# heli-sudoo/HKD-MPC

Hardware: AMD Instinct MI355X
Metric: batched DDP iters/sec (fwd+bwd), 4-phase 200-knot HKD fp64, batch=4096 (higher is better)
Workload: dtype f64

## Files before the change

### hkd-mpc_amd/csrc/hkd_model.h

```cpp
#pragma once

#ifndef __HIPCC__
#ifndef __host__
#define __host__
#define __device__
#endif
#endif
#include <math.h>

#define HKD_FN __host__ __device__ inline

namespace hkd {

constexpr int NX = 24;
constexpr int NU = 24;
constexpr int SE_N = 15;
constexpr int SW_N = 51;
constexpr int BW_N = 36;

constexpr double kMass = 8.9120000000000008e+00;
constexpr double kGravity = -9.8100000000000005e+00;
constexpr double kI00 = 2.7460779999999994e-02, kI01 = 1.0842021724855044e-19, kI02 = -1.2037062152420224e-35;
constexpr double kI11 = 2.4251579680000002e-01, kI22 = 2.6519357680000000e-01;
constexpr double kJ00 = 3.6415571589736352e+01, kJ01 = -1.6280111378663628e-17, kJ02 = 1.6528925920107902e-33;
// ... 96 lines not shown
    contact_moment(x, u, c, w);
#pragma unroll
    for (int i = 0; i < 3; ++i) tau[i] = R.r[0][i] * w[0] + R.r[1][i] * w[1] + R.r[2][i] * w[2];
    inertia_apply(om, Iw);
    rhs[0] = tau[0] - (om[1] * Iw[2] - om[2] * Iw[1]);
    rhs[1] = tau[1] - (om[2] * Iw[0] - om[0] * Iw[2]);
    rhs[2] = tau[2] - (om[0] * Iw[1] - om[1] * Iw[0]);
    inertia_inv_apply(rhs, acc);
#pragma unroll
    for (int i = 0; i < 3; ++i) xn[6 + i] = om[i] + dt * acc[i];
#pragma unroll
    for (int i = 0; i < 3; ++i) {
        double f = c[0] * u[i] + c[1] * u[3 + i] + c[2] * u[6 + i] + c[3] * u[9 + i];
        xn[9 + i] = x[9 + i] + dt * (f / kMass + (i == 2 ? kGravity : 0.0));
    }
#pragma unroll
    for (int l = 0; l < 4; ++l)
#pragma unroll
        for (int j = 0; j < 3; ++j) xn[12 + 3 * l + j] = x[12 + 3 * l + j] + (1.0 - c[l]) * u[12 + 3 * l + j] * dt;
}

HKD_FN void hkd_partial_compact(const double *x, const double *u, const double *c, double dt, double *Se,
                                double *Sw, double *Bw)
{
    const double *om = x + 6;
    const EulTrig tr = eul_trig(x);
    const double cp = tr.cp, sp = tr.sp, cr = tr.cr, sr = tr.sr;
    double a = sr * om[1] + cr * om[2], b = cr * om[1] - sr * om[2];
    const double icp = 1.0 / cp, tp = sp * icp;
    Se[0] = dt * a * sp * (icp * icp); Se[1] = dt * b * icp; Se[2] = 0.0; Se[3] = dt * sr * icp; Se[4] = dt * cr * icp;
    Se[5] = 0.0;                     Se[6] = -dt * a;     Se[7] = 0.0;     Se[8] = dt * cr;      Se[9] = -dt * sr;
    Se[10] = dt * a * icp * icp;     Se[11] = dt * tp * b; Se[12] = dt;    Se[13] = dt * sr * tp; Se[14] = dt * cr * tp;
    Rot R, Dy, Dp, Dr;
    rot_zyx(tr, R);
    rot_zyx_grad(tr, Dy, Dp, Dr);
    double w[3];
    contact_moment(x, u, c, w);
    double M[3][17];
#pragma unroll
    for (int i = 0; i < 3; ++i) {
        M[i][0] = Dy.r[0][i] * w[0] + Dy.r[1][i] * w[1] + Dy.r[2][i] * w[2];
        M[i][1] = Dp.r[0][i] * w[0] + Dp.r[1][i] * w[1] + Dp.r[2][i] * w[2];
        M[i][2] = Dr.r[0][i] * w[0] + Dr.r[1][i] * w[1] + Dr.r[2][i] * w[2];
#pragma unroll
        for (int q = 3; q < 17; ++q) M[i][q] = 0.0;
    }
#pragma unroll
    for (int l = 0; l < 4; ++l) {
        const double *f = u + 3 * l;
        double Sf[3][3] = {{0.0, -f[2], f[1]}, {f[2], 0.0, -f[0]}, {-f[1], f[0], 0.0}};
#pragma unroll
        for (int i = 0; i < 3; ++i)
#pragma unroll
            for (int k = 0; k < 3; ++k) {
                double t = c[l] * (R.r[0][i] * Sf[0][k] + R.r[1][i] * Sf[1][k] + R.r[2][i] * Sf[2][k]);
                M[i][3 + k] += t;
                if (k < 2) M[i][9 + 2 * l + k] = -t;
            }
    }
    double Iw[3];
    inertia_apply(om, Iw);
    const double Ssk[3][3] = {{0.0, -Iw[2], Iw[1]}, {Iw[2], 0.0, -Iw[0]}, {-Iw[1], Iw[0], 0.0}};
    const double So[3][3] = {{0.0, -om[2], om[1]}, {om[2], 0.0, -om[0]}, {-om[1], om[0], 0.0}};
    const double In[3][3] = {{kI00, kI01, kI02}, {kI01, kI11, 0.0}, {kI02, 0.0, kI22}};
#pragma unroll
    for (int i = 0; i < 3; ++i)
#pragma unroll
        for (int k = 0; k < 3; ++k)
            M[i][6 + k] = Ssk[i][k] - (So[i][0] * In[0][k] + So[i][1] * In[1][k] + So[i][2] * In[2][k]);
#pragma unroll
    for (int q = 0; q < 17; ++q) {
        double v[3] = {M[0][q], M[1][q], M[2][q]}, o[3];
        inertia_inv_apply(v, o);
        Sw[q] = dt * o[0]; Sw[17 + q] = dt * o[1]; Sw[34 + q] = dt * o[2];
    }
#pragma unroll
    for (int l = 0; l < 4; ++l) {
        double r0 = x[12 + 3 * l] - x[3], r1 = x[13 + 3 * l] - x[4], r2 = -x[5];
        double Sr[3][3] = {{0.0, -r2, r1}, {r2, 0.0, -r0}, {-r1, r0, 0.0}};
#pragma unroll
        for (int k = 0; k < 3; ++k) {
            double v[3], o[3];
#pragma unroll
            for (int i = 0; i < 3; ++i) v[i] = c[l] * (R.r[0][i] * Sr[0][k] + R.r[1][i] * Sr[1][k] + R.r[2][i] * Sr[2][k]);
            inertia_inv_apply(v, o);
            Bw[3 * l + k] = dt * o[0]; Bw[12 + 3 * l + k] = dt * o[1]; Bw[24 + 3 * l + k] = dt * o[2];
        }
    }
}

template <typename Emit>
HKD_FN void hkd_partial_emit(const double *x, const double *u, const double *c, double dt, Emit emit)
{
    const double *om = x + 6;
    const EulTrig tr = eul_trig(x);
    const double cp = tr.cp, sp = tr.sp, cr = tr.cr, sr = tr.sr;
    double a = sr * om[1] + cr * om[2], b = cr * om[1] - sr * om[2];
    const double icp = 1.0 / cp, tp = sp * icp;
    emit(0, 0, dt * a * sp * (icp * icp)); emit(0, 1, dt * b * icp); emit(0, 2, 0.0); emit(0, 3, dt * sr * icp);
    emit(0, 4, dt * cr * icp); emit(0, 5, 0.0); emit(0, 6, -dt * a); emit(0, 7, 0.0); emit(0, 8, dt * cr);
    emit(0, 9, -dt * sr); emit(0, 10, dt * a * icp * icp); emit(0, 11, dt * tp * b); emit(0, 12, dt);
    emit(0, 13, dt * sr * tp); emit(0, 14, dt * cr * tp);
    Rot R, Dy, Dp, Dr;
    rot_zyx(tr, R);
    rot_zyx_grad(tr, Dy, Dp, Dr);
    auto col = [&](const double (&v)[3], int q) {
        double o[3];
        inertia_inv_apply(v, o);
        emit(1, q, dt * o[0]); emit(1, 17 + q, dt * o[1]); emit(1, 34 + q, dt * o[2]);
    };
    {
        double w[3];
        contact_moment(x, u, c, w);
        double v[3];
#pragma unroll
        for (int i = 0; i < 3; ++i) v[i] = Dy.r[0][i] * w[0] + Dy.r[1][i] * w[1] + Dy.r[2][i] * w[2];
        col(v, 0);
#pragma unroll
        for (int i = 0; i < 3; ++i) v[i] = Dp.r[0][i] * w[0] + Dp.r[1][i] * w[1] + Dp.r[2][i] * w[2];
        col(v, 1);
#pragma unroll
        for (int i = 0; i < 3; ++i) v[i] = Dr.r[0][i] * w[0] + Dr.r[1][i] * w[1] + Dr.r[2][i] * w[2];
        col(v, 2);
    }
    auto tl = [&](int l, int i, int k) {
        const double *f = u + 3 * l;
        const double Sf[3][3] = {{0.0, -f[2], f[1]}, {f[2], 0.0, -f[0]}, {-f[1], f[0], 0.0}};
        return c[l] * (R.r[0][i] * Sf[0][k] + R.r[1][i] * Sf[1][k] + R.r[2][i] * Sf[2][k]);
    };
#pragma unroll
    for (int k = 0; k < 3; ++k) {
        double v[3] = {0.0, 0.0, 0.0};
#pragma unroll
        for (int l = 0; l < 4; ++l)
#pragma unroll
            for (int i = 0; i < 3; ++i) v[i] += tl(l, i, k);
        col(v, 3 + k);
    }
    {
        double Iw[3];
        inertia_apply(om, Iw);
        const double Ssk[3][3] = {{0.0, -Iw[2], Iw[1]}, {Iw[2], 0.0, -Iw[0]}, {-Iw[1], Iw[0], 0.0}};
        const double So[3][3] = {{0.0, -om[2], om[1]}, {om[2], 0.0, -om[0]}, {-om[1], om[0], 0.0}};
        const double In[3][3] = {{kI00, kI01, kI02}, {kI01, kI11, 0.0}, {kI02, 0.0, kI22}};
#pragma unroll
        for (int k = 0; k < 3; ++k) {
            double v[3];
#pragma unroll
            for (int i = 0; i < 3; ++i) v[i] = Ssk[i][k] - (So[i][0] * In[0][k] + So[i][1] * In[1][k] + So[i][2] * In[2][k]);
            col(v, 6 + k);
        }
    }
#pragma unroll
    for (int l = 0; l < 4; ++l)
#pragma unroll
        for (int k = 0; k < 2; ++k) {
            double v[3];
#pragma unroll
            for (int i = 0; i < 3; ++i) v[i] = -tl(l, i, k);
            col(v, 9 + 2 * l + k);
        }
#pragma unroll
    for (int l = 0; l < 4; ++l) {
        double r0 = x[12 + 3 * l] - x[3], r1 = x[13 + 3 * l] - x[4], r2 = -x[5];
        double Sr[3][3] = {{0.0, -r2, r1}, {r2, 0.0, -r0}, {-r1, r0, 0.0}};
#pragma unroll
        for (int k = 0; k < 3; ++k) {
            double v[3], o[3];
#pragma unroll
            for (int i = 0; i < 3; ++i) v[i] = c[l] * (R.r[0][i] * Sr[0][k] + R.r[1][i] * Sr[1][k] + R.r[2][i] * Sr[2][k]);
            inertia_inv_apply(v, o);
            emit(2, 3 * l + k, dt * o[0]); emit(2, 12 + 3 * l + k, dt * o[1]); emit(2, 24 + 3 * l + k, dt * o[2]);
        }
    }
}

HKD_FN void hkd_expand_colmajor(const double *Se, const double *Sw, const double *Bw, const double *c, double dt,
                                double *A, double *B)
{
    for (int i = 0; i < NX * NX; ++i) { A[i] = 0.0; B[i] = 0.0; }
    for (int i = 0; i < NX; ++i) A[i + NX * i] = 1.0;
    for (int r = 0; r < 3; ++r)
        for (int q = 0; q < 5; ++q) A[r + NX * se_col(q)] += Se[5 * r + q];
    for (int i = 0; i < 3; ++i) A[(3 + i) + NX * (9 + i)] = dt;
    for (int r = 0; r < 3; ++r)
        for (int q = 0; q < 17; ++q) A[(6 + r) + NX * sw_col(q)] += Sw[17 * r + q];
    for (int r = 0; r < 3; ++r)
        for (int k = 0; k < 12; ++k) B[(6 + r) + NX * k] = Bw[12 * r + k];
    for (int l = 0; l < 4; ++l)
        for (int j = 0; j < 3; ++j) {
            B[(9 + j) + NX * (3 * l + j)] = dt * c[l] / kMass;
            B[(12 + 3 * l + j) + NX * (12 + 3 * l + j)] = dt * (1.0 - c[l]);
        }
}

HKD_FN void foot_body_trig(int l, const double *tr, double *pb, double (*dpb)[3])
{
    double s = leg_side(l), f = leg_front(l);
    const double s0 = tr[0], c0 = tr[1], s1 = tr[2], c1 = tr[3], s12 = tr[4], c12 = tr[5];
    pb[0] = kHipX * f - kLower * s12 - kUpper * s1;
    pb[1] = kSideY * s + kAbad * s * c0 - kLower * s0 * c12 - kUpper * s0 * c1;
    pb[2] = kLower * c0 * c12 + kUpper * c0 * c1 + kAbad * s * s0;
    if (dpb) {
        dpb[0][0] = 0.0; dpb[0][1] = -kLower * c12 - kUpper * c1; dpb[0][2] = -kLower * c12;
        dpb[1][0] = -kAbad * s * s0 - kLower * c0 * c12 - kUpper * c0 * c1;
        dpb[1][1] = kLower * s0 * s12 + kUpper * s0 * s1; dpb[1][2] = kLower * s0 * s12;
        dpb[2][0] = -kLower * s0 * c12 - kUpper * s0 * c1 + kAbad * s * c0;
        dpb[2][1] = -kLower * c0 * s12 - kUpper * c0 * s1; dpb[2][2] = -kLower * c0 * s12;
    }
}

HKD_FN void foot_body(int l, const double *q, double *pb, double (*dpb)[3])
{
    double tr[6];
    sincos(q[0], &tr[0], &tr[1]);
    sincos(q[1], &tr[2], &tr[3]);
    sincos(q[1] + q[2], &tr[4], &tr[5]);
    foot_body_trig(l, tr, pb, dpb);
}

HKD_FN void hkd_foot_position(int l, const double *pos, const double *eul, const double *q, double *p)
{
    Rot R;
    rot_zyx(eul, R);
    double pb[3];
    foot_body(l, q, pb, nullptr);
    for (int i = 0; i < 3; ++i) p[i] = pos[i] + R.r[i][0] * pb[0] + R.r[i][1] * pb[1] + R.r[i][2] * pb[2];
}

HKD_FN void hkd_foot_jacobian(int l, const double *eul, const double *q, double *J)
{
    Rot R, Dy, Dp, Dr;
    const EulTrig tr = eul_trig(eul);
    rot_zyx(tr, R);
    rot_zyx_grad(tr, Dy, Dp, Dr);
    double pb[3], dpb[3][3];
    foot_body(l, q, pb, dpb);
    for (int i = 0; i < 54; ++i) J[i] = 0.0;
    for (int i = 0; i < 3; ++i) {
        J[18 * i + i] = 1.0;
        J[18 * i + 3] = Dy.r[i][0] * pb[0] + Dy.r[i][1] * pb[1] + Dy.r[i][2] * pb[2];
        J[18 * i + 4] = Dp.r[i][0] * pb[0] + Dp.r[i][1] * pb[1] + Dp.r[i][2] * pb[2];
        J[18 * i + 5] = Dr.r[i][0] * pb[0] + Dr.r[i][1] * pb[1] + Dr.r[i][2] * pb[2];
        for (int k = 0; k < 3; ++k)
            J[18 * i + 6 + 3 * l + k] = R.r[i][0] * dpb[0][k] + R.r[i][1] * dpb[1][k] + R.r[i][2] * dpb[2][k];
    }
}

__host__ __device__ __forceinline__ double hkd_foot_height_grad(int l, const double *x, double *hx)
{
    Rot R, Dy, Dp, Dr;
    const EulTrig tr = eul_trig(x);
    rot_zyx(tr, R);
    rot_zyx_grad(tr, Dy, Dp, Dr);
    double pb[3], dpb[3][3];
    foot_body(l, x + 12 + 3 * l, pb, dpb);
    if (hx) {
        for (int j = 0; j < NX; ++j) hx[j] = 0.0;
        hx[0] = Dy.r[2][0] * pb[0] + Dy.r[2][1] * pb[1] + Dy.r[2][2] * pb[2];
        hx[1] = Dp.r[2][0] * pb[0] + Dp.r[2][1] * pb[1] + Dp.r[2][2] * pb[2];
        hx[2] = Dr.r[2][0] * pb[0] + Dr.r[2][1] * pb[1] + Dr.r[2][2] * pb[2];
        hx[5] = 1.0;
        for (int k = 0; k < 3; ++k)
            hx[12 + 3 * l + k] = R.r[2][0] * dpb[0][k] + R.r[2][1] * dpb[1][k] + R.r[2][2] * dpb[2][k];
    }
    return x[5] + R.r[2][0] * pb[0] + R.r[2][1] * pb[1] + R.r[2][2] * pb[2];
}

HKD_FN double hkd_foot_height_grad_sparse(int l, const double *x, double *ge, double *gq)
{
    Rot R, Dy, Dp, Dr;
    const EulTrig tr = eul_trig(x);
    rot_zyx(tr, R);
    rot_zyx_grad(tr, Dy, Dp, Dr);
    double pb[3], dpb[3][3];
    foot_body(l, x + 12 + 3 * l, pb, dpb);
    ge[0] = Dy.r[2][0] * pb[0] + Dy.r[2][1] * pb[1] + Dy.r[2][2] * pb[2];
    ge[1] = Dp.r[2][0] * pb[0] + Dp.r[2][1] * pb[1] + Dp.r[2][2] * pb[2];
    ge[2] = Dr.r[2][0] * pb[0] + Dr.r[2][1] * pb[1] + Dr.r[2][2] * pb[2];
    for (int k = 0; k < 3; ++k) gq[k] = R.r[2][0] * dpb[0][k] + R.r[2][1] * dpb[1][k] + R.r[2][2] * dpb[2][k];
    return x[5] + R.r[2][0] * pb[0] + R.r[2][1] * pb[1] + R.r[2][2] * pb[2];
}

HKD_FN void hkd_resetmap(const double *x, const int *c, const int *cn, double *xn)
{
    for (int j = 0; j < NX; ++j) xn[j] = x[j];
#pragma unroll
    for (int l = 0; l < 4; ++l) {
        if (c[l] && !cn[l]) { xn[12 + 3 * l] = 0.0; xn[13 + 3 * l] = -0.8; xn[14 + 3 * l] = 1.7; }
        if (!c[l] && cn[l]) {
            double p[3];
            hkd_foot_position(l, x + 3, x, x + 12 + 3 * l, p);
            xn[12 + 3 * l] = p[0]; xn[13 + 3 * l] = p[1]; xn[14 + 3 * l] = 0.0 * p[2];
        }
    }
}

HKD_FN void hkd_resetmap_partial_row(const double *x, const int *c, const int *cn, int r, double *row)
{
    for (int j = 0; j < NX; ++j) row[j] = (j == r) ? 1.0 : 0.0;
    if (r < 12) return;
    int l = (r - 12) / 3, k = (r - 12) % 3;
    if (c[l] && !cn[l]) { row[r] = 0.0; return; }
    if (!c[l] && cn[l]) {
        row[r] = 0.0;
        if (k == 2) return;
        double J[54];
        hkd_foot_jacobian(l, x, x + 12 + 3 * l, J);
        for (int j = 0; j < 3; ++j) { row[j] = J[18 * k + 3 + j]; row[3 + j] = J[18 * k + j]; }
        for (int j = 0; j < 12; ++j) row[12 + j] = J[18 * k + 6 + j];
    }
}

}
```

### hkd-mpc_amd/csrc/hsddp_api.cpp

```cpp
#include <algorithm>
#include <cmath>
#include <cstddef>
#include <cstdio>
#include <cstdlib>
#include <cstring>

#include "hsddp_handle.h"
#include "hsddp_measure.h"
#include "hsddp_simulate.h"

using namespace hsddp;

static thread_local std::string g_err;

int hsddp::fail(int code, const std::string &msg)
{
    g_err = msg;
    return code;
}

extern "C" int hsddp_ref_fail(int code, const char *msg) { return fail(code, msg); }

extern "C" const char *hsddp_last_error(void) { return g_err.c_str(); }
extern "C" const char *hsddp_version(void) { return "hsddp-mi355x 0.1 (gfx950, fp64)"; }

static void fill_params(hsddp_handle h)
{
    h->slots_fresh = false;
    Params &p = h->p;
    const hsddp_problem_desc &ds = h->desc;
    const hsddp_options &o = h->opt;
    p.dt = ds.dt;
    p.dt_m = ds.dt / hkd::kMass;
    {
        const char *tr = std::getenv("HSDDP_TRACE");
        p.trace = (tr && tr[0] == '1') ? 1 : 0;
    }
    p.mu = ds.cparams.mu_fric;
    p.grf_delta = ds.cparams.grf_delta; p.grf_delta_min = ds.cparams.grf_delta_min; p.grf_eps = ds.cparams.grf_eps;
    p.td_sigma = ds.cparams.td_sigma; p.td_sigma_max = ds.cparams.td_sigma_max; p.td_lambda = ds.cparams.td_lambda;
    p.ground = ds.cparams.ground_height;
    const hsddp_hkd_weights &w = ds.weights;
    for (int j = 0; j < 3; ++j) { p.qbase[j] = w.q_eul[j]; p.qbase[3 + j] = w.q_pos[j]; p.qbase[6 + j] = w.q_omega[j]; p.qbase[9 + j] = w.q_v[j]; }
    p.q_qJ = w.q_qJ;
    for (int j = 0; j < 24; ++j) p.qf_scale[j] = w.qf_scale[j];
    p.qf_gain = w.qf_gain; p.r_grf = w.r_grf; p.r_qJd = w.r_qJd;
    for (int j = 0; j < 3; ++j) p.foot_w[j] = w.foot_w[j];
    p.foot_gain = w.foot_gain; p.foot_term_cost = w.foot_term_cost; p.foot_term_grad = w.foot_term_grad;
    p.alpha = o.alpha; p.gamma = o.gamma; p.update_penalty = o.update_penalty; p.update_relax = o.update_relax;
    p.update_regularization = o.update_regularization; p.update_ReB = o.update_ReB;
    p.cost_thresh = o.cost_thresh; p.tconstr_thresh = o.tconstr_thresh; p.pconstr_thresh = o.pconstr_thresh;
    p.feas_thresh = o.dynamics_feas_thresh; p.merit_scale = o.merit_scale; p.merit_offset = o.merit_offset;
    p.AL_active = o.AL_active; p.ReB_active = o.ReB_active; p.no_early_exit = o.no_early_exit;
    p.ms0 = o.MS ? 0 : 1;
    p.reb_uniform = o.update_ReB == 1.0 && o.update_relax == 1.0 && p.grf_delta >= p.grf_delta_min && h->reb_at_init;
    p.grf_inv_delta = 1.0 / p.grf_delta;
    p.grf_log_delta = std::log(p.grf_delta);
    int M = 0;
    if (o.update_regularization > 1) {
        double mu = 0;
        for (;;) {
            mu = std::fmax(mu * o.update_regularization, 1e-03);
            if (mu > 1e2) break;
            if (++M > 64) { M = 0; break; }
        }
    }
    p.retry_m = M;
    p.retry_cap = (M > 0 && M <= h->retry_m_alloc && !p.store_value && p.B >= 4) ? h->retry_cap_alloc : 0;
}

static int ensure_history(hsddp_handle h)
{
    const long need = std::max(1 + (long)std::max(0, h->opt.max_AL_iter) * std::max(0, h->opt.max_DDP_iter),
                               h->budgets_on ? 1 + h->bud_hist : 0L);
    if (h->hist && need <= h->p.hcap) return HSDDP_OK;
    const int cap = (int)std::min<long>(std::max<long>(need, 16), 1 << 20);
    float *nh = nullptr;
    HIPCHK(hipMalloc(&nh, (size_t)h->p.B * cap * 4 * sizeof(float)));
    HIPCHK(hipMemset(nh, 0, (size_t)h->p.B * cap * 4 * sizeof(float)));
    HIPCHK(hipStreamSynchronize(nullptr));
    if (h->hist) {
        HIPCHK(hipStreamSynchronize(h->stream));
        hipFree(h->hist);
        h->bytes -= (size_t)h->p.B * h->p.hcap * 4 * sizeof(float);
    }
    h->hist = nh;
    h->d.hist = nh;
    h->p.hcap = cap;
    h->bytes += (size_t)h->p.B * cap * 4 * sizeof(float);
    return HSDDP_OK;
}

extern "C" int hsddp_create(const hsddp_problem_desc *desc, hsddp_handle *out)
{
    if (!desc || !out) return fail(HSDDP_ERR_ARG, "null argument");
    if (desc->batch < 1 || desc->n_phases < 1 || desc->n_phases > HSDDP_MAX_PHASES || !(desc->dt > 0))
        return fail(HSDDP_ERR_ARG, "invalid batch / n_phases / dt");
    Layout L0;
    std::string why;
    if (int rc = build_layout(desc->n_phases, desc->horizons, nullptr, L0, why)) return fail(rc, why);
    int ndev = 0;
    if (hipGetDeviceCount(&ndev) != hipSuccess || ndev < 1)
        return fail(HSDDP_ERR_DEVICE, "no HIP device available (the solver has no CPU fallback)");
    if (desc->device < 0 || desc->device >= ndev) return fail(HSDDP_ERR_DEVICE, "device ordinal out of range");
    HIPCHK(hipSetDevice(desc->device));
    hsddp_handle h = new hsddp_handle_t();
    h->desc = *desc;
    hsddp_default_options(&h->opt);
    Params &p = h->p;
    p.B = desc->batch;
    p.Kc = control_slots(L0);
    p.ref_per_element = desc->ref_per_element ? 1 : 0;
    p.fp32 = desc->riccati_fp32 ? 1 : 0;
    h->Bref = p.ref_per_element ? p.B : 1;
    adopt_shared_layout(h, L0, nullptr);
    fill_params(h);
    h->S_cap = (size_t)p.Kc + HSDDP_MAX_PHASES;
    const size_t B = p.B, S = h->S_cap, Kc = p.Kc, P = HSDDP_MAX_PHASES, Br = h->Bref;
    Bufs &d = h->d;
    int *contacts; double *x0, *rx, *ru, *rf;
    int rc = 0;
    if ((rc = dalloc(h, contacts, B * (P + 1) * 4)) || (rc = dalloc(h, x0, B * NX)) || (rc = dalloc(h, rx, Br * S * NX)) ||
        (rc = dalloc(h, ru, Br * S * NX)) || (rc = dalloc(h, rf, Br * S * 12)) || (rc = dalloc(h, d.ref_t, REF_COLS * Br * S)) ||
        (rc = dalloc(h, d.X3, 3 * B * S * NX)) ||
        (rc = dalloc(h, d.D3, 3 * B * S * NX)) || (rc = dalloc(h, d.U3, 3 * B * Kc * NX)) || (rc = dalloc(h, d.sel, B)) ||
        (rc = dalloc(h, d.cf_u, B * Kc * 12)) || (rc = dalloc(h, d.cf_flag, B * Kc)) ||
        (rc = dalloc(h, d.dX, B * S * NX)) ||
        (rc = dalloc(h, d.dU, B * Kc * NX)) ||
        (rc = dalloc(h, d.du, B * Kc * NX)) || (rc = dalloc(h, d.dbg, B * 16)) ||
        (p.fp32 ? ((rc = dalloc(h, d.K32, B * Kc * KCW)) || (rc = dalloc(h, d.lq32, B * Kc * LQW32)) ||
                   (rc = dalloc(h, d.def32, B * S * NX)))
                : ((rc = dalloc(h, d.K, B * Kc * KCW)) || (rc = dalloc(h, d.lq, B * Kc * LQW)))) ||
        (rc = dalloc(h, d.term, B * P * TW)) || (rc = dalloc(h, d.reb_delta, B * Kc * 20)) ||
        (rc = dalloc(h, d.reb_eps, B * Kc * 20)) || (rc = dalloc(h, d.al_sigma, B * P * MTD * 4)) ||
        (rc = dalloc(h, d.al_lambda, B * P * MTD * 4)) || (rc = dalloc(h, d.td_mask, B * P * MTD)) ||
        (rc = dalloc(h, d.term_h, B * P * 4)) ||
        (rc = dalloc(h, d.slot_cost, B * S)) || (rc = dalloc(h, d.slot_feas, B * S)) || (rc = dalloc(h, d.slot_viol, B * S)) ||
        (rc = dalloc(h, d.slot_div, B * S)) || (rc = dalloc(h, d.el, B)) || (rc = dalloc(h, d.counter, 8)) || (rc = dalloc(h, d.ls_live, LS_LIVE)) ||
        (rc = dalloc(h, (Layout *&)d.lay, B)) || (rc = dalloc(h, (int *&)d.pairs, 2 * B + 2))) {
        hsddp_destroy(h);
        return rc;
    }
    d.contacts = contacts; d.x0 = x0; d.ref_x = rx; d.ref_u = ru; d.ref_foot = rf;
    d.ref_tw = Br * S;
    d.xs3 = B * S * NX;
    d.us3 = B * Kc * NX;
    d.rows3 = (int)(B * S);
    d.urows3 = (int)(B * Kc);
    {
        const char *seq = std::getenv("HSDDP_SEQUENTIAL_RETRY");
        const char *capenv = std::getenv("HSDDP_RETRY_CAP");
        const size_t per_elem = (size_t)std::max(1, p.retry_m) * Kc * (KCW * (p.fp32 ? 4 : 8) + NX * 8 + 4);
        size_t cap = std::min<size_t>(std::min<size_t>(128, B), std::max<size_t>(2, ((size_t)256 << 20) / per_elem));
        if (capenv && std::atoi(capenv) > 0) cap = std::min<size_t>(cap, (size_t)std::atoi(capenv));
        const size_t M = (seq && seq[0] == '1') ? 0 : p.retry_m, n = cap * M;
        if (M > 0) {
            void *rk;
            if ((rc = dalloc(h, d.retry_list, cap)) || (rc = dalloc(h, d.retry_count, 1)) ||
                (rc = dalloc(h, d.retry_flag, n)) || (rc = dalloc(h, d.retry_dU, n * Kc * NX)) ||
                (rc = dalloc(h, d.retry_dv, n)) ||
                (rc = p.fp32 ? dalloc(h, (float *&)rk, n * Kc * KCW) : dalloc(h, (double *&)rk, n * Kc * KCW))) {
                hsddp_destroy(h);
                return rc;
            }
            d.retry_K = rk;
            h->retry_cap_alloc = (int)cap;
            h->retry_m_alloc = (int)M;
            fill_params(h);
        }
    }
    if (hipStreamCreateWithFlags(&h->stream, hipStreamNonBlocking) != hipSuccess ||
        hipHostMalloc((void **)&h->host_counter, 16 * sizeof(int), 0) != hipSuccess) {
        hsddp_destroy(h);
        return fail(HSDDP_ERR_DEVICE, "stream / pinned allocation failed");
    }
    if ((rc = ensure_history(h))) {
        hsddp_destroy(h);
        return rc;
    }
    launch_init_params(p, d, h->stream);
    launch_reset_elements(p, d, h->stream);
    if (hipStreamSynchronize(h->stream) != hipSuccess) {
        hsddp_destroy(h);
        return fail(HSDDP_ERR_DEVICE, "kernel launch failed at create (is the library built for this GPU?)");
    }
    *out = h;
    return HSDDP_OK;
}

// ... 848 lines not shown
}

extern "C" int hsddp_download_trajectory(hsddp_handle h, double *Xbar, double *Ubar, double *K)
{
    if (!h) return fail(HSDDP_ERR_ARG, "null handle");
    HIPCHK(hipSetDevice(h->desc.device));
    HIPCHK(hipStreamSynchronize(h->stream));
    const size_t B = h->p.B, S = h->p.S, Kc = h->p.Kc;
    int rc;
    launch_normalize(h->p, h->d, h->stream);
    HIPCHK(hipStreamSynchronize(h->stream));
    if ((rc = d2h(Xbar, h->d.X3, B * S * NX * 8)) || (rc = d2h(Ubar, h->d.U3, B * Kc * NX * 8)))
        return rc;
    if (K && h->need_inputs)
        return fail(HSDDP_ERR_ARG, "the layout changed (hsddp_shift): call hsddp_update_problem before downloading K");
    if (K) {
        std::vector<double> kc(B * Kc * KCW);
        if (h->p.fp32) {
            std::vector<float> k32(B * Kc * KCW);
            if ((rc = d2h(k32.data(), h->d.K32, B * Kc * KCW * 4))) return rc;
            std::copy(k32.begin(), k32.end(), kc.begin());
        } else if ((rc = d2h(kc.data(), h->d.K, B * Kc * KCW * 8))) {
            return rc;
        }
        std::memset(K, 0, B * Kc * NN * sizeof(double));
        for (size_t b = 0; b < B; ++b)
            for (size_t k = 0; k < Kc; ++k)
                for (int q = 0; q < 12; ++q) {
                    const int u = coupled_control(h, b, k, q);
                    std::memcpy(K + ((b * Kc + k) * NX + u) * NX, &kc[((b * Kc + k) * 12 + q) * NX], NX * sizeof(double));
                }
    }
    return HSDDP_OK;
}

extern "C" int hsddp_debug_stamps(hsddp_handle h, unsigned long long *out)
{
    if (!h || !out) return fail(HSDDP_ERR_ARG, "null argument");
    HIPCHK(hipSetDevice(h->desc.device));
    HIPCHK(hipStreamSynchronize(h->stream));
    HIPCHK(hipMemcpy(out, h->d.dbg, h->p.B * 16 * sizeof(unsigned long long), hipMemcpyDeviceToHost));
    return HSDDP_OK;
}

extern "C" int hsddp_download_working(hsddp_handle h, double *X, double *U, double *Defect, double *dX, double *dU)
{
    if (!h) return fail(HSDDP_ERR_ARG, "null handle");
    HIPCHK(hipSetDevice(h->desc.device));
    HIPCHK(hipStreamSynchronize(h->stream));
    const size_t B = h->p.B, S = h->p.S, Kc = h->p.Kc;
    int rc;
    if ((rc = d2h(dX, h->d.dX, B * S * NX * 8)) || (rc = d2h(dU, h->d.dU, B * Kc * NX * 8)))
        return rc;
    if (X || U || Defect) {
        std::vector<int> sel(B);
        HIPCHK(hipMemcpy(sel.data(), h->d.sel, B * sizeof(int), hipMemcpyDeviceToHost));
        for (int q = 0; q < 3; ++q) {
            std::vector<double> xb(X ? B * S * NX : 0), ub(U ? B * Kc * NX : 0), db(Defect ? B * S * NX : 0);
            if ((rc = d2h(X ? xb.data() : nullptr, h->d.X3 + q * h->d.xs3, B * S * NX * 8)) ||
                (rc = d2h(U ? ub.data() : nullptr, h->d.U3 + q * h->d.us3, B * Kc * NX * 8)) ||
                (rc = d2h(Defect ? db.data() : nullptr, h->d.D3 + q * h->d.xs3, B * S * NX * 8)))
                return rc;
            for (size_t b = 0; b < B; ++b) {
                if (((sel[b] >> 2) & 3) != q) continue;
                if (X) std::copy(xb.begin() + b * S * NX, xb.begin() + (b + 1) * S * NX, X + b * S * NX);
                if (U) std::copy(ub.begin() + b * Kc * NX, ub.begin() + (b + 1) * Kc * NX, U + b * Kc * NX);
                if (Defect) std::copy(db.begin() + b * S * NX, db.begin() + (b + 1) * S * NX, Defect + b * S * NX);
            }
        }
    }
    return HSDDP_OK;
}

extern "C" int hsddp_download_references(hsddp_handle h, double *ref_x, double *ref_u, double *ref_foot)
{
    if (!h || !ref_x || !ref_u || !ref_foot) return fail(HSDDP_ERR_ARG, "null argument");
    HIPCHK(hipSetDevice(h->desc.device));
    HIPCHK(hipStreamSynchronize(h->stream));
    const size_t Br = h->Bref, S = h->p.S;
    int rc;
    if ((rc = d2h(ref_x, h->d.ref_x, Br * S * NX * 8)) || (rc = d2h(ref_u, h->d.ref_u, Br * S * NX * 8)) ||
        (rc = d2h(ref_foot, h->d.ref_foot, Br * S * 12 * 8)))
        return rc;
    return HSDDP_OK;
}

extern "C" int hsddp_download_element_info(hsddp_handle h, hsddp_element_info *info)
{
    if (!h || !info) return fail(HSDDP_ERR_ARG, "null argument");
    HIPCHK(hipSetDevice(h->desc.device));
    HIPCHK(hipStreamSynchronize(h->stream));
    std::vector<ElemState> el(h->p.B);
    HIPCHK(hipMemcpy(el.data(), h->d.el, h->p.B * sizeof(ElemState), hipMemcpyDeviceToHost));
    for (int b = 0; b < h->p.B; ++b) {
        const ElemState &e = el[b];
        info[b].cost = e.cost; info[b].feas = e.feas; info[b].merit = e.merit;
        info[b].max_tconstr = e.max_t; info[b].max_pconstr = e.max_p;
        info[b].iters = e.iters; info[b].outer_iters = e.outer_iters; info[b].status = e.status;
        info[b].n_ls_trials = e.n_ls;
    }
    return HSDDP_OK;
}

extern "C" int hsddp_download_solver_info(hsddp_handle h, int capacity, float *cost, float *dyn_feas,
                                          float *eqn_feas, float *ineq_feas, int *count)
{
    if (!h || capacity < 0) return fail(HSDDP_ERR_ARG, "null handle or negative capacity");
    HIPCHK(hipSetDevice(h->desc.device));
    HIPCHK(hipStreamSynchronize(h->stream));
    const int B = h->p.B, hc = h->p.hcap;
    std::vector<ElemState> el(B);
    HIPCHK(hipMemcpy(el.data(), h->d.el, B * sizeof(ElemState), hipMemcpyDeviceToHost));
    std::vector<float> hv((size_t)B * hc * 4);
    HIPCHK(hipMemcpy(hv.data(), h->d.hist, hv.size() * sizeof(float), hipMemcpyDeviceToHost));
    float *outs[4] = {cost, dyn_feas, eqn_feas, ineq_feas};
    for (int b = 0; b < B; ++b) {
        const int n = std::min(el[b].hist_n, std::min(hc, capacity));
        if (count) count[b] = n;
        for (int f = 0; f < 4; ++f) {
            if (!outs[f]) continue;
            float *o = outs[f] + (size_t)b * capacity;
            for (int k = 0; k < capacity; ++k) o[k] = k < n ? hv[((size_t)b * hc + k) * 4 + f] : 0.0f;
        }
    }
    return HSDDP_OK;
}



extern "C" int hsddp_download_lq(hsddp_handle h, double *A, double *Bm, double *l, double *lx, double *lu,
                                 double *lxx, double *luu)
{
    if (!h) return fail(HSDDP_ERR_ARG, "null handle");
    HIPCHK(hipSetDevice(h->desc.device));
    HIPCHK(hipStreamSynchronize(h->stream));
    const Params &p = h->p;
    const size_t B = p.B, Kc = p.Kc, S = p.S, W = p.fp32 ? LQW32 : LQW;
    std::vector<double> rec(B * Kc * W), cost(B * S);
    if (p.fp32) {
        std::vector<float> r32(B * Kc * W);
        HIPCHK(hipMemcpy(r32.data(), h->d.lq32, r32.size() * sizeof(float), hipMemcpyDeviceToHost));
        for (size_t q = 0; q < rec.size(); ++q) rec[q] = r32[q];
    } else {
        HIPCHK(hipMemcpy(rec.data(), h->d.lq, rec.size() * sizeof(double), hipMemcpyDeviceToHost));
    }
    if (l) HIPCHK(hipMemcpy(cost.data(), h->d.slot_cost, cost.size() * sizeof(double), hipMemcpyDeviceToHost));
    const double dt = p.dt;
    for (size_t b = 0; b < B; ++b)
        for (size_t kc = 0; kc < Kc; ++kc) {
            const double *r = rec.data() + (b * Kc + kc) * W;
            const int i = phase_of_control(layout_of(h, b), (int)kc);
            const int *c = h->contacts.data() + (b * (p.P + 1) + i) * 4;
            const size_t o = (b * Kc + kc);
            if (A) {
                double *a = A + o * NN;
                std::fill(a, a + NN, 0.0);
                for (int j = 0; j < NX; ++j) a[j * NX + j] = 1.0;
                for (int rr = 0; rr < 3; ++rr)
                    for (int q = 0; q < 5; ++q) a[rr * NX + hkd::se_col(q)] += r[LQ_SE + 5 * rr + q];
                for (int q = 0; q < 3; ++q) a[(3 + q) * NX + 9 + q] += dt;
                for (int rr = 0; rr < 3; ++rr)
                    for (int q = 0; q < 17; ++q) a[(6 + rr) * NX + hkd::sw_col(q)] += r[sw_at(rr, q)];
            }
            if (Bm) {
                double *bb = Bm + o * NN;
                std::fill(bb, bb + NN, 0.0);
                for (int rr = 0; rr < 3; ++rr)
                    for (int q = 0; q < 12; ++q) bb[(6 + rr) * NX + q] = r[bw_at(rr, q)];
                for (int lg = 0; lg < 4; ++lg)
                    for (int a = 0; a < 3; ++a) {
                        bb[(9 + a) * NX + 3 * lg + a] = dt * c[lg] / hkd::kMass;
                        bb[(12 + 3 * lg + a) * NX + 12 + 3 * lg + a] = dt * (1.0 - c[lg]);
                    }
            }
            Wts wr;
            weights_row(weights_of(h, b), wr);
            if (l) l[o] = cost[b * S + kc + i];
            if (lx) for (int j = 0; j < NX; ++j) lx[o * NX + j] = r[LQ_LX + j];
            if (lu) for (int j = 0; j < NX; ++j) lu[o * NX + j] = r[LQ_LU + j];
            if (lxx) {
                double *m = lxx + o * NN;
                std::fill(m, m + NN, 0.0);
                for (int j = 0; j < NX; ++j)
                    m[j * NX + j] = dt * (j < 12 ? wr.qbase[j] : wr.q_qJ * (1 - c[(j - 12) / 3]));
                for (int lg = 0; lg < 4; ++lg)
                    for (int a = 0; a < 3; ++a) {
                        const double w = c[lg] ? dt * (wr.foot_gain * wr.foot_w[a]) : 0.0;
                        const int pa = 3 + a, qa = 12 + 3 * lg + a;
                        m[pa * NX + pa] += w; m[qa * NX + qa] += w;
                        m[pa * NX + qa] -= w; m[qa * NX + pa] -= w;
                    }
            }
            if (luu) {
                double *m = luu + o * NN;
                std::fill(m, m + NN, 0.0);
                for (int j = 0; j < NX; ++j) m[j * NX + j] = dt * (j < 12 ? wr.r_grf : wr.r_qJd);
                static const int ix[3][3] = {{0, 1, 2}, {1, 3, 4}, {2, 4, 5}};
                for (int lg = 0; lg < 4; ++lg)
                    for (int a = 0; a < 3; ++a)
                        for (int e = 0; e < 3; ++e) m[(3 * lg + a) * NX + 3 * lg + e] += r[LQ_RB + 6 * lg + ix[a][e]];
            }
        }
    return HSDDP_OK;
}

extern "C" int hsddp_download_terminal(hsddp_handle h, double *Phi, double *Phix, double *Phixx, double *Px)
{
    if (!h) return fail(HSDDP_ERR_ARG, "null handle");
    HIPCHK(hipSetDevice(h->desc.device));
    HIPCHK(hipStreamSynchronize(h->stream));
    const Params &p = h->p;
    const size_t B = p.B, P = p.P;
    std::vector<double> term(B * P * TW), cost(B * p.S);
    HIPCHK(hipMemcpy(term.data(), h->d.term, term.size() * sizeof(double), hipMemcpyDeviceToHost));
    HIPCHK(hipMemcpy(cost.data(), h->d.slot_cost, cost.size() * sizeof(double), hipMemcpyDeviceToHost));
    for (size_t b = 0; b < B; ++b) {
        const Layout L = layout_of(h, b);
        for (size_t i = 0; i < P; ++i) {
            const double *t = term.data() + (b * P + i) * TW;
            const size_t o = b * P + i;
            if ((int)i >= L.P) {
                if (Phi) Phi[o] = 0;
                if (Phix) std::fill(Phix + o * NX, Phix + (o + 1) * NX, 0.0);
                if (Phixx) std::fill(Phixx + o * NN, Phixx + (o + 1) * NN, 0.0);
                if (Px) std::fill(Px + o * NN, Px + (o + 1) * NN, 0.0);
                continue;
            }
            if (Phi) Phi[o] = cost[b * p.S + L.s0[i] + L.N[i]];
            if (Phix) std::copy(t + TM_PHIX, t + TM_PHIX + NX, Phix + o * NX);
            if (Phixx) std::copy(t + TM_PHIXX, t + TM_PHIXX + NN, Phixx + o * NN);
            if (Px) {
                if ((int)i + 1 < L.P) std::copy(t + TM_PX, t + TM_PX + NN, Px + o * NN);
                else std::fill(Px + o * NN, Px + (o + 1) * NN, 0.0);
            }
        }
    }
    return HSDDP_OK;
}

extern "C" int hsddp_set_value_export(hsddp_handle h, int on)
{
    if (!h) return fail(HSDDP_ERR_ARG, "null handle");
    HIPCHK(hipSetDevice(h->desc.device));
    if (on && !h->value0) {
        const size_t n = (size_t)h->p.B * HSDDP_MAX_PHASES * (NX + NN);
        HIPCHK(hipMalloc(&h->value0, n * sizeof(double)));
        HIPCHK(hipMemset(h->value0, 0, n * sizeof(double)));
        HIPCHK(hipStreamSynchronize(nullptr));
        h->bytes += n * sizeof(double);
        h->d.value0 = h->value0;
    }
    h->p.store_value = on ? 1 : 0;
    fill_params(h);
    return HSDDP_OK;
}

extern "C" int hsddp_download_value(hsddp_handle h, double *G, double *H)
{
    if (!h) return fail(HSDDP_ERR_ARG, "null handle");
    if (!h->value0 || !h->p.store_value) return fail(HSDDP_ERR_ARG, "value export is off (hsddp_set_value_export)");
    HIPCHK(hipSetDevice(h->desc.device));
    HIPCHK(hipStreamSynchronize(h->stream));
    const size_t B = h->p.B, P = h->p.P;
    std::vector<double> v(B * P * (NX + NN));
    HIPCHK(hipMemcpy(v.data(), h->value0, v.size() * sizeof(double), hipMemcpyDeviceToHost));
    for (size_t o = 0; o < B * P; ++o) {
        const bool live = (int)(o % P) < layout_of(h, o / P).P;
        const double *s = v.data() + o * (NX + NN);
        if (G) { if (live) std::copy(s, s + NX, G + o * NX); else std::fill(G + o * NX, G + (o + 1) * NX, 0.0); }
        if (H) { if (live) std::copy(s + NX, s + NX + NN, H + o * NN); else std::fill(H + o * NN, H + (o + 1) * NN, 0.0); }
    }
    return HSDDP_OK;
}

extern "C" int hsddp_synchronize(hsddp_handle h)
{
    if (!h) return fail(HSDDP_ERR_ARG, "null handle");
    HIPCHK(hipStreamSynchronize(h->stream));
    return HSDDP_OK;
}

extern "C" size_t hsddp_device_bytes(hsddp_handle h) { return h ? h->bytes : 0; }

static int check_launch()
{
    HIPCHK(hipGetLastError());
    return HSDDP_OK;
}

extern "C" int hsddp_hkd_dynamics(const double *x, const double *u, const double *c, double dt, double *xn, int n,
                                  void *stream)
{
    if (!x || !u || !c || !xn || n < 0) return fail(HSDDP_ERR_ARG, "bad argument");
    if (n) launch_model_dynamics(x, u, c, dt, xn, n, (hipStream_t)stream);
    return check_launch();
}
extern "C" int hsddp_hkd_dynamics_partial(const double *x, const double *u, const double *c, double dt, double *A,
                                          double *B, int n, void *stream)
{
    if (!x || !u || !c || !A || !B || n < 0) return fail(HSDDP_ERR_ARG, "bad argument");
    if (n) launch_model_partial(x, u, c, dt, A, B, n, (hipStream_t)stream);
    return check_launch();
}
extern "C" int hsddp_hkd_foot_position(const double *x, const int *leg, double *p, int n, void *stream)
{
    if (!x || !leg || !p || n < 0) return fail(HSDDP_ERR_ARG, "bad argument");
    if (n) launch_model_foot(x, leg, p, nullptr, n, (hipStream_t)stream);
    return check_launch();
}
extern "C" int hsddp_hkd_state(const hsddp_robot_state *states, const int *contact, double *x, int n, void *stream)
{
    if (!states || !contact || !x || n < 0) return fail(HSDDP_ERR_ARG, "bad argument");
    if (n) launch_hkd_state(states, contact, 4, x, n, (hipStream_t)stream);
    return check_launch();
}
extern "C" int hsddp_hkd_foot_jacobian(const double *x, const int *leg, double *J, int n, void *stream)
{
    if (!x || !leg || !J || n < 0) return fail(HSDDP_ERR_ARG, "bad argument");
    if (n) launch_model_foot(x, leg, nullptr, J, n, (hipStream_t)stream);
    return check_launch();
}
extern "C" int hsddp_hkd_resetmap(const double *x, const int *c, const int *cn, double *xn, int n, void *stream)
{
    if (!x || !c || !cn || !xn || n < 0) return fail(HSDDP_ERR_ARG, "bad argument");
    if (n) launch_model_reset(x, c, cn, xn, nullptr, n, (hipStream_t)stream);
    return check_launch();
}
extern "C" int hsddp_hkd_resetmap_partial(const double *x, const int *c, const int *cn, double *Px, int n,
                                          void *stream)
{
    if (!x || !c || !cn || !Px || n < 0) return fail(HSDDP_ERR_ARG, "bad argument");
    if (n) launch_model_reset(x, c, cn, nullptr, Px, n, (hipStream_t)stream);
    return check_launch();
}

static Params plugin_params(const hsddp_hkd_weights &w, double dt)
{
    Params p{};
    p.dt = dt;
    for (int j = 0; j < 3; ++j) { p.qbase[j] = w.q_eul[j]; p.qbase[3 + j] = w.q_pos[j]; p.qbase[6 + j] = w.q_omega[j]; p.qbase[9 + j] = w.q_v[j]; }
    p.q_qJ = w.q_qJ;
    for (int j = 0; j < 24; ++j) p.qf_scale[j] = w.qf_scale[j];
    p.qf_gain = w.qf_gain; p.r_grf = w.r_grf; p.r_qJd = w.r_qJd;
    for (int j = 0; j < 3; ++j) p.foot_w[j] = w.foot_w[j];
    p.foot_gain = w.foot_gain; p.foot_term_cost = w.foot_term_cost; p.foot_term_grad = w.foot_term_grad;
    return p;
}
extern "C" int hsddp_hkd_running_cost(const double *x, const double *u, const int *c, const double *xr, const double *ur,
                                      const double *pf, const hsddp_hkd_weights *w, double dt, int terms, double *l,
                                      double *lx, double *lu, double *lxx, double *luu, int n, void *stream)
{
    if (!x || !u || !c || !xr || !ur || !pf || !w || n < 0 || (terms & ~3)) return fail(HSDDP_ERR_ARG, "bad argument");
    if (n) launch_model_running_cost(plugin_params(*w, dt), x, u, c, xr, ur, pf, terms, l, lx, lu, lxx, luu, n,
// ... 56 lines not shown
```

### hkd-mpc_amd/csrc/hsddp_internal.h

```cpp
#pragma once

#include <hip/hip_runtime.h>
#include <cstddef>
#include "hkd_model.h"
#include "hsddp_phases.h"

namespace hsddp {

constexpr int NX = 24;
constexpr int NN = 576;
constexpr int LS_LIVE = 128;
constexpr int MTD = 4;
constexpr int TD_PENDING = 0x10;
constexpr int KCW = 12 * 24;

constexpr int LQ_SE = 0;
constexpr int LQ_SW = 16;
constexpr int LQ_BW = 68;
constexpr int LQ_LX = 104;
constexpr int LQ_LU = 128;
constexpr int LQ_RB = 152;
constexpr int LQW = 176;
constexpr int LQW32 = 192;
constexpr int sw_at(int r, int q) { return LQ_SW + 3 * q + r; }
constexpr int bw_at(int r, int k) { return LQ_BW + 3 * k + r; }
static_assert(LQ_SE + 15 < LQ_SW && LQ_SW + 51 < LQ_BW && LQ_BW + 36 == LQ_LX && LQ_LX + 24 == LQ_LU &&
              LQ_LU + 24 == LQ_RB && LQ_RB + 24 == LQW, "record layout");

constexpr int MAX_REG_ATTEMPTS = 64;

constexpr int TM_PHIX = 0;
constexpr int TM_PHIXX = 32;
constexpr int TM_PX = TM_PHIXX + NN;
constexpr int TW = TM_PX + NN;
static_assert(TM_PHIXX % 16 == 0 && TM_PX % 16 == 0 && TW % 16 == 0, "terminal record lines");


struct Params {
    int B, P, S, Kc;
    int N[MAXP], s0[MAXP], k0[MAXP];
    int ref_per_element;
    double dt, dt_m , mu, grf_delta, grf_delta_min, grf_eps, td_sigma, td_sigma_max, td_lambda, ground;
    double qbase[12], q_qJ, qf_scale[24], qf_gain, r_grf, r_qJd, foot_w[3], foot_gain, foot_term_cost, foot_term_grad;
    double alpha, gamma, update_penalty, update_relax, update_regularization, update_ReB;
    double cost_thresh, tconstr_thresh, pconstr_thresh, feas_thresh, merit_scale, merit_offset;
    int AL_active, ReB_active, no_early_exit;
    int reb_uniform;
    double grf_inv_delta, grf_log_delta;
    int lq_slots;
    int fp32;
    int ss[MAXP];
    int has_tail;
    int retry_cap, retry_m;
    int hcap;
    int elem_layout;
    int n_pairs;
    int store_value;
    int ms0;
    int trace;
};

struct Wts {
    double qbase[12], q_qJ, qf_scale[24], qf_gain, r_grf, r_qJd, foot_w[3], foot_gain, foot_term_cost, foot_term_grad;
    double pad[2];
};
static_assert(sizeof(Wts) == 48 * sizeof(double), "Wts: three 128-byte lines");
static_assert(offsetof(Params, foot_term_grad) - offsetof(Params, qbase) == offsetof(Wts, foot_term_grad),
              "Wts: Params' weight fields in Params' order");

struct RetryEntry {
    int b, pad;
    double reg;
};

constexpr int TD_STALE = 0x20;

struct ElemState {
    double cost, feas, merit, merit_rho, dV1, dV2, reg;
    double max_t, max_p, max_t_prev, max_p_prev, cost_prev, merit_prev, feas_prev;
    int done, inner_done, ls_active, accepted, status, iters, outer_iters, n_ls;
    int hist_n;
    int ovr, td_stale;
    int inner_n;
};
static_assert(sizeof(ElemState) == 160, "ElemState: 14 doubles and 12 ints, no padding left");


struct Bufs {
    const int *contacts;
    const double *x0;
    const double *ref_x, *ref_u, *ref_foot;
    double *ref_t;
    size_t ref_tw;
    double *X3, *D3, *dX;
    double *U3, *dU, *du;
    size_t xs3, us3;
    int rows3, urows3;
    int *sel;
    double *cf_u;
    int *cf_flag;
    double *K, *lq, *term;
    double *reb_delta, *reb_eps, *al_sigma, *al_lambda, *term_h;
    int *td_mask;
    double *slot_cost, *slot_feas, *slot_viol;
    int *slot_div;
    float *lq32, *K32, *def32;
    ElemState *el;
    int *counter;
    int *ls_live;
    RetryEntry *retry_list;
    int *retry_count, *retry_flag;
    void *retry_K;
    double *retry_dU;
    double *retry_dv;
    unsigned long long *dbg;
    float *hist;
    const Layout *lay;
    const int *pairs;
    double *value0;
};


void launch_lq(const Params &p, const Bufs &d, const double *terrain, const Wts *weights, hipStream_t st);

void launch_riccati(const Params &p, const Bufs &d, const Wts *weights, hipStream_t st);
void launch_lin_rollout(const Params &p, const Bufs &d, const Wts *weights, hipStream_t st);

void launch_rollout(const Params &p, const Bufs &d, double eps, int last, int init, int tix, const int *budget,
                    const double *terrain, const Wts *weights, hipStream_t st);
void launch_decide(const Params &p, const Bufs &d, double eps, int last, int init, int tix, const int *budget,
                   const double *terrain, const Wts *weights, hipStream_t st);

void launch_normalize(const Params &p, const Bufs &d, hipStream_t st);
void launch_reset_working(const Params &p, const Bufs &d, hipStream_t st);
void launch_outer_begin(const Params &p, const Bufs &d, const int *budget, hipStream_t st);
void launch_reb_update(const Params &p, const Bufs &d, const double *terrain, hipStream_t st);
void launch_outer_end(const Params &p, const Bufs &d, const int *budget, hipStream_t st);
void launch_reset_elements(const Params &p, const Bufs &d, hipStream_t st);
void launch_init_params(const Params &p, const Bufs &d, hipStream_t st);
void launch_resolve_td(const Params &p, const Bufs &d, hipStream_t st);
void launch_upload_td(const Params &p, const Bufs &d, const int *legs, hipStream_t st);
constexpr int REF_COLS = 24 + 24 + 12;
void launch_ref_columns(const Params &p, const Bufs &d, int Bref, hipStream_t st);
void launch_count(const Params &p, const Bufs &d, int which, hipStream_t st);
void launch_stat_sums(const Params &p, const Bufs &d, hipStream_t st);
void launch_broadcast(double *dst, const double *src, size_t n, size_t copies, hipStream_t st);

void launch_model_dynamics(const double *x, const double *u, const double *c, double dt, double *xn, int n,
                           hipStream_t st);
void launch_model_partial(const double *x, const double *u, const double *c, double dt, double *A, double *B,
                          int n, hipStream_t st);
void launch_model_foot(const double *x, const int *leg, double *p, double *J, int n, hipStream_t st);
void launch_model_reset(const double *x, const int *c, const int *cn, double *xn, double *Px, int n,
                        hipStream_t st);
void launch_model_running_cost(const Params &p, const double *x, const double *u, const int *c, const double *xr,
                               const double *ur, const double *pf, int terms, double *l, double *lx, double *lu,
                               double *lxx, double *luu, int n, hipStream_t st);
void launch_model_terminal_cost(const Params &p, const double *x, const int *c, const double *xr, const double *pf,
                                int terms, double *Phi, double *Phix, double *Phixx, int n, hipStream_t st);
void launch_model_grf(const double *u, const int *c, double mu, double *g, double *gu, int n, hipStream_t st);
void launch_model_touchdown(const double *x, const int *c, const int *cn, double ground, double *h, double *hx, int n,
                            hipStream_t st);

}
```

### hkd-mpc_amd/csrc/hsddp_linear.hip

```cpp
#include "hsddp_wave.h"
#include "hsddp_dispatch.h"

namespace hsddp {

using namespace hkd;

constexpr int HC = 12;

#ifndef HSDDP_STAMPS
#define HSDDP_STAMPS 0
#endif
#if HSDDP_STAMPS
struct LinStamps {
    unsigned long long st[8], tprev;
};
DEV LinStamps &lin_stamps()
{
    __shared__ LinStamps s;
    return s;
}
#define LSTAMP(n)                                                                             \
    do {                                                                                      \
        __builtin_amdgcn_sched_barrier(0);                                                    \
        unsigned long long t_;                                                                \
        asm volatile("s_waitcnt lgkmcnt(0)\n\ts_memtime %0\n\ts_waitcnt lgkmcnt(0)" : "=s"(t_)::"memory"); \
        __builtin_amdgcn_sched_barrier(0);                                                    \
        if (threadIdx.x == 0) {                                                               \
            if ((n) > 0) lin_stamps().st[n] += t_ - lin_stamps().tprev;                       \
            lin_stamps().tprev = t_;                                                          \
        }                                                                                     \
    } while (0)
#else
#define LSTAMP(n) \
    do {          \
    } while (0)
#endif

template <typename real> struct Prec;
template <> struct Prec<double> {
    static constexpr int LQS = LQW;
    static DEV const double *lq(const Bufs &d) { return d.lq; }
    static DEV double *K(const Bufs &d) { return d.K; }
    static DEV const double *def(const Bufs &d, int b) { return kdbuf(work_buf(d, b)); }
};
template <> struct Prec<float> {
    static constexpr int LQS = LQW32;
    static DEV const float *lq(const Bufs &d) { return d.lq32; }
    static DEV float *K(const Bufs &d) { return d.K32; }
    static DEV const float *def(const Bufs &d, int) { return d.def32; }
};

template <typename real>
struct PhaseConst {
    int c[4];
    int cmask;
    real bv[4];
    real bq[4];
};

template <typename real>
DEV void load_phase(const Params &p, const Bufs &d, const size_t (&b)[2], int hf, int i, PhaseConst<real> &pc)
{
    typedef const __attribute__((address_space(4))) int cint;
    cint *c0 = (cint *)(d.contacts + (b[0] * (p.P + 1) + i) * 4), *c1 = (cint *)(d.contacts + (b[1] * (p.P + 1) + i) * 4);
    pc.cmask = 0;
#pragma unroll
    for (int l = 0; l < 4; ++l) {
        const int a0 = c0[l], a1 = c1[l];
        pc.c[l] = hf ? a1 : a0;
        pc.cmask |= (pc.c[l] != 0) << l;
        pc.bv[l] = pc.c[l] ? (real)p.dt_m : (real)0;
        pc.bq[l] = pc.c[l] ? (real)0 : (real)p.dt;
    }
}

template <typename real>
struct LxxRow {
    real diag, xq[4], xp;
};

template <typename real>
DEV int contact(const PhaseConst<real> &pc, int l) { return (pc.cmask >> l) & 1; }

template <typename T>
DEV T pick4(const T (&a)[4], int i)
{
    return i == 0 ? a[0] : i == 1 ? a[1] : i == 2 ? a[2] : a[3];
}

template <int N>
DEV double pick(const double (&a)[N], int i)
{
    double e[N];
#pragma unroll
    for (int k = 0; k < N; ++k) {
        e[k] = a[k];
        asm volatile("" : "+s"(e[k]));
    }
    double v = e[0];
#pragma unroll
    for (int k = 1; k < N; ++k) v = i == k ? e[k] : v;
    return v;
}

template <typename real, typename WT>
DEV void lxx_row(const Params &p, const WT &ww, const PhaseConst<real> &pc, int r, LxxRow<real> &L)
{
    auto at = [&](const auto &a, int i) {
        if constexpr (std::is_same_v<WT, Params>) return pick(a, i);
        else return a[i];
    };
    L.diag = 0.0; L.xp = 0.0;
#pragma unroll
    for (int l = 0; l < 4; ++l) L.xq[l] = 0.0;
    if (r >= NX) return;
    double dg = p.dt * (r < 12 ? at(ww.qbase, r) : ww.q_qJ * (1 - contact(pc, (r - 12) / 3)));
    if (r >= 3 && r < 6) {
        const double fw = p.dt * (ww.foot_gain * at(ww.foot_w, r - 3));
#pragma unroll
        for (int l = 0; l < 4; ++l) {
            const double w = pc.c[l] ? fw : 0.0;
            dg += w;
            L.xq[l] = -w;
        }
    } else if (r >= 12) {
        const int m = r - 12;
        const double w = contact(pc, m / 3) ? p.dt * (ww.foot_gain * at(ww.foot_w, m % 3)) : 0.0;
        dg += w;
        L.xp = -w;
    }
    L.diag = dg;
}

template <typename real>
struct LinImg {
    static constexpr int K = 0;
    static constexpr int LQ = K + KCW * (int)sizeof(real);
    static constexpr int D = LQ + Prec<real>::LQS * (int)sizeof(real);
    static constexpr int DU = D + NX * (int)sizeof(real);
    static constexpr int END = DU + NX * 8;
    static constexpr int NI = (END / 16 + 63) / 64;
    static_assert(LQ % 16 == 0 && D % 16 == 0 && DU % 16 == 0 && END % 16 == 0 && (NI == 4 || NI == 3), "16-byte pieces");
};
template <typename real>
struct LinBuf {
    alignas(16) char v[2][LinImg<real>::NI * 1024];
};
constexpr int LZ = 31;
template <typename real>
struct LinVec {
    real dx[2][32], du[2][32];
    real zero[64];
};

template <typename real>
struct LinSrc {
    using I = LinImg<real>;
    const char *p[2][I::NI];
    unsigned step[I::NI];

    static DEV int piece(int j, int lane)
    {
        const int o = 16 * (64 * j + lane);
        return o < I::END ? o : I::END - 16;
    }
    DEV void init(const Params &pr, const Bufs &d, const size_t (&b)[2], int s, int kc, int lane)
    {
#pragma unroll
        for (int j = 0; j < I::NI; ++j) {
            const int o = piece(j, lane);
            step[j] = o < I::LQ ? KCW * sizeof(real) : o < I::D ? Prec<real>::LQS * sizeof(real) : o < I::DU ? NX * sizeof(real) : NX * 8;
#pragma unroll
            for (int h = 0; h < 2; ++h) {
                const size_t kq = b[h] * pr.Kc + kc;
                const char *base = o < I::LQ ? (const char *)(Prec<real>::K(d) + kq * KCW) - I::K
                                 : o < I::D  ? (const char *)(Prec<real>::lq(d) + kq * Prec<real>::LQS) - I::LQ
                                 : o < I::DU ? (const char *)(Prec<real>::def(d, (int)b[h]) + (b[h] * pr.S + s + 1) * NX) - I::D
                                             : (const char *)(d.dU + kq * NX) - I::DU;
                p[h][j] = base + o;
            }
        }
    }
    DEV void advance()
    {
#pragma unroll
        for (int j = 0; j < I::NI; ++j) {
            p[0][j] += step[j];
            p[1][j] += step[j];
        }
    }
};

template <typename real>
DEV void lin_fetch(LinBuf<real> &buf, const LinSrc<real> &src)
{
#pragma unroll
    for (int h = 0; h < 2; ++h)
#pragma unroll
        for (int j = 0; j < LinImg<real>::NI; ++j)
            lds_dma16_nt(src.p[h][j], (unsigned)(size_t)(buf.v[h] + 1024 * j));
}

template <int W>
DEV void vm_wait()
{
    if constexpr (W == 0) asm volatile("s_waitcnt vmcnt(0)" ::: "memory");
    else if constexpr (W == 2) asm volatile("s_waitcnt vmcnt(2)" ::: "memory");
    else if constexpr (W == 6) asm volatile("s_waitcnt vmcnt(6)" ::: "memory");
    else if constexpr (W == 8) asm volatile("s_waitcnt vmcnt(8)" ::: "memory");
    else if constexpr (W == 10) asm volatile("s_waitcnt vmcnt(10)" ::: "memory");
    else if constexpr (W == 4) asm volatile("s_waitcnt vmcnt(4)" ::: "memory");
    else if constexpr (W == 12) asm volatile("s_waitcnt vmcnt(12)" ::: "memory");
    else static_assert(W < 0, "wait count");
}

template <int NI2>
DEV void vm_wait_n(int n)
{
    if (n == NI2 + 4) vm_wait<NI2 + 4>();
    else if (n == NI2 + 2) vm_wait<NI2 + 2>();
    else if (n == NI2) vm_wait<NI2>();
    else if (n == 4) vm_wait<4>();
    else if (n == 2) vm_wait<2>();
    else vm_wait<0>();
}

template <typename real>
struct LinRow {
    PhaseConst<real> pc;
    LxxRow<real> lx;
    real ru;
    bool cpl;
    int krow0;
    bool use_se, use_sw, use_rb;
    int se0, sw0, rb0, rbi[3];
    real c3;
    int i3;
    real cx[4];
    int ix[4];
    real cu[4];
    int iu[4];
    real cq;
    int iru;
};

template <typename real>
DEV void lin_row(const Params &p, LinRow<real> &R, int r)
{
    const int rr = r < NX ? r : 0;
    R.use_se = r < 3;
    R.use_sw = r >= 6 && r < 9;
    R.use_rb = r < 12;
    R.se0 = LQ_SE + 5 * (r < 3 ? r : 0);
    R.sw0 = r >= 6 && r < 9 ? r - 6 : 0;
    R.rb0 = LQ_RB + 6 * ((r < 12 ? r : 0) / 3);
    const int a = (r < 12 ? r : 0) % 3;
#pragma unroll
    for (int b = 0; b < 3; ++b) R.rbi[b] = a == 0 ? b : a == 1 ? (b == 0 ? 1 : b == 1 ? 3 : 4) : (b == 0 ? 2 : b == 1 ? 4 : 5);
    R.iru = r < 12 ? 3 * (r / 3) : LZ;
    R.c3 = (r >= 3 && r < 6) ? (real)p.dt : (real)0;
    R.i3 = (r >= 3 && r < 6) ? r + 6 : LZ;
#pragma unroll
    for (int l = 0; l < 4; ++l) {
        const bool pos = r >= 3 && r < 6, q = r >= 12 && r < NX;
        R.cx[l] = pos ? R.lx.xq[l] : (q && l == 0) ? R.lx.xp : (real)0;
        R.ix[l] = pos ? 12 + 3 * l + r - 3 : (q && l == 0) ? 3 + (r - 12) % 3 : LZ;
        const bool v = r >= 9 && r < 12;
        R.cu[l] = v ? R.pc.bv[l] : (real)0;
        R.iu[l] = v ? 3 * l + r - 9 : LZ;
    }
    R.cq = (r >= 12 && r < NX) ? pick4(R.pc.bq, (rr - 12) / 3) : (real)0;
}

template <typename real>
struct LinOut {
    double *du, *dx;
    real vu, vx;
    int n;
    int nprev;
    bool ust;
};

template <typename real>
DEV void lin_push(LinOut<real> &out, real du, real nx)
{
    out.vu = du;
    out.vx = nx;
    out.n = 1;
}

template <typename real>
DEV int lin_store_pending(bool go, bool st, LinOut<real> &out)
{
    if (!go || out.n == 0) return 0;
    out.n = 0;
    if (st) {
        if (out.ust) *out.du = (double)out.vu;
        *out.dx = (double)out.vx;
    }
    out.du += NX;
    out.dx += NX;
    return 2;
}

template <typename real>
DEV void lin_knot(const Params &p, LinVec<real> &S, LinBuf<real> &cur, LinBuf<real> &nxt, bool more, bool pend,
                  LinSrc<real> &src, const LinRow<real> &R, bool st, LinOut<real> &out, real &dx, real &q1s, real &q2s)
{
    using I = LinImg<real>;
    constexpr int NI2 = 2 * I::NI;
    const int lane = threadIdx.x, r = lane & 31, hf = lane >> 5;
    const bool rowl = r < NX;
    const int rr = rowl ? r : 0;
    LSTAMP(0);
    if (more) {
        src.advance();
        lin_fetch(nxt, src);
    }
    const int ns = lin_store_pending(pend, st, out);
    vm_wait_n<NI2>(out.nprev + (more ? NI2 : 0) + ns);
    out.nprev = ns;
    LSYNC();
    LSTAMP(1);
    const char *img = cur.v[hf];
    const real *kimg = (const real *)(img + I::K), *lq = (const real *)(img + I::LQ), *dd = (const real *)(img + I::D);
    const double *dUi = (const double *)(img + I::DU);
    real *sdxv = S.dx[hf], *sduv = S.du[hf];
    const real *kp = R.cpl ? kimg + R.krow0 : S.zero;
    const real *sep = R.use_se ? lq + R.se0 : S.zero, *swp = R.use_sw ? lq + LQ_SW + R.sw0 : S.zero;
    const real *bwp = R.use_sw ? lq + LQ_BW + R.sw0 : S.zero, *rbp = R.use_rb ? lq + R.rb0 : S.zero;
    const real *lxp = rowl ? lq + LQ_LX : S.zero, *lup = rowl ? lq + LQ_LU : S.zero;
    real krow[NX], cse[5], csw[17], cbw[12], crb[3];
#pragma unroll
    for (int c = 0; c < NX; ++c) krow[c] = kp[c];
    const real dUr = (real)dUi[rr];
#pragma unroll
    for (int q = 0; q < 5; ++q) cse[q] = sep[5 * 0 + q];
#pragma unroll
    for (int q = 0; q < 17; ++q) csw[q] = swp[3 * q];
    const real ddr = (rowl ? dd : S.zero)[rr], lxr = lxp[rr], lur = lup[rr];
    if (rowl) sdxv[r] = dx;
    real dxa, dxb;
    row_pair(dx, dxa, dxb);
    asm volatile("" : "+v"(dxa), "+v"(dxb));
    asm volatile("s_nop 1");
    pin(krow);
    real k0 = 0, k1 = 0;
    static_for<HC>([&](auto C) {
        constexpr int c = C, c1 = HC + C;
        bfma<c>(k0, dxa, krow[c]);
        if constexpr (c1 < 16) bfma<c1>(k1, dxa, krow[c1]);
        else bfma<c1 - 16>(k1, dxb, krow[c1]);
    });
    const real du = dUr + (k0 + k1);
    LSTAMP(2);
    SFENCE();
#pragma unroll
    for (int q = 0; q < 12; ++q) cbw[q] = bwp[3 * q];
#pragma unroll
    for (int b = 0; b < 3; ++b) crb[b] = rbp[R.rbi[b]];
    if (rowl) sduv[r] = du;
    const real x3 = sdxv[R.i3];
    real xc[4];
#pragma unroll
    for (int l = 0; l < 4; ++l) xc[l] = sdxv[R.ix[l]];
    pin(cse);
    pin(csw);
    real se = 0, sw = 0;
    static_for<5>([&](auto Q) { bfma<se_col(Q)>(se, dxa, cse[Q]); });
    static_for<17>([&](auto Q) {
        constexpr int col = sw_col(Q);
        if constexpr (col < 16) bfma<col>(sw, dxa, csw[Q]);
        else bfma<col - 16>(sw, dxb, csw[Q]);
    });
    real dua, dub;
    row_pair(du, dua, dub);
    asm volatile("" : "+v"(dua), "+v"(dub));
    asm volatile("s_nop 1");
    pin(cbw);
    real bw = 0;
    static_for<12>([&](auto C) { bfma<C>(bw, dua, cbw[C]); });
    (void)dub;
    LSYNC();
    LSTAMP(3);
    real uc[4], ur[3];
#pragma unroll
    for (int l = 0; l < 4; ++l) uc[l] = sduv[R.iu[l]];
#pragma unroll
    for (int b = 0; b < 3; ++b) ur[b] = sduv[R.iru < LZ ? R.iru + b : LZ];
    const real sdx = (se + sw) + R.c3 * x3;
    real lxd = R.lx.diag * dx;
#pragma unroll
    for (int l = 0; l < 4; ++l) lxd += R.cx[l] * xc[l];
    real bdu = bw;
#pragma unroll
    for (int l = 0; l < 4; ++l) bdu += R.cu[l] * uc[l];
    bdu += R.cq * du;
    const real lud = R.ru * du + (crb[0] * ur[0] + crb[1] * ur[1] + crb[2] * ur[2]);
    const real nx = rowl ? ((dx + sdx) + bdu) + ddr : (real)0;
    q1s += lxr * dx + lur * du;
    q2s += dx * lxd + du * lud;
    lin_push(out, du, nx);
    dx = nx;
    LSYNC();
    LSTAMP(4);
}

template <typename real, bool EL, typename... WP>
__global__ __launch_bounds__(64, 2) void k_lin_rollout(Params p, Bufs d, WP... wp)
{
    const auto wt = terrain_of(wp...);
    __shared__ LinVec<real> S;
    __shared__ LinBuf<real> B0;
    __shared__ LinBuf<real> B1;
    const int lane = threadIdx.x, r = lane & 31, hf = lane >> 5;
    size_t eb[2];
    bool valid;
    if constexpr (EL) {
        const int e0 = d.pairs[2 * blockIdx.x], e1 = d.pairs[2 * blockIdx.x + 1];
        eb[0] = e0;
        eb[1] = e1 >= 0 ? e1 : e0;
        valid = hf == 0 || e1 >= 0;
    } else {
        const int e0 = 2 * blockIdx.x, e1 = e0 + 1;
        eb[0] = e0;
        eb[1] = e1 < p.B ? e1 : e0;
        valid = hf == 0 || e1 < p.B;
    }
    const size_t b = hf ? eb[1] : eb[0];
    ElemState &E = d.el[b];
    const bool act = valid && !E.done && !E.inner_done;
    if (!__builtin_amdgcn_ballot_w64(act)) return;
    const bool rowl = r < NX, st = rowl && act;
    const int rr = rowl ? r : 0;
    const real *defg = Prec<real>::def(d, (int)b);
    S.zero[lane] = 0;
    S.dx[hf][r] = 0;
    S.du[hf][r] = 0;
#if HSDDP_STAMPS
    if (lane < 8) lin_stamps().st[lane] = 0;
#endif
    __syncthreads();
    real v1 = 0, v2 = 0, dx = 0;
    const auto LY = layout_of<EL>(d, (int)eb[0]);
    const int P = LY.P();
    LinOut<real> out{};
    for (int i = 0; i < P; ++i) {
        const int N = LY.N(i), s0 = LY.s0(i), k0 = LY.k0(i);
        LinSrc<real> src;
        src.init(p, d, eb, s0, k0, lane);
        lin_fetch(B0, src);
        out.nprev = 0;
        LinRow<real> R;
        load_phase(p, d, eb, hf, i, R.pc);
        if (i > 0) {
            const double *Px = d.term + (b * p.P + (i - 1)) * TW + TM_PX;
            if (rowl) S.dx[hf][r] = dx;
            LSYNC();
            real a = 0;
            if (rowl)
                for (int j = 0; j < NX; ++j) a += (real)Px[r * NX + j] * S.dx[hf][j];
            dx = a;
            LSYNC();
        } else {
            dx = 0;
        }
        if (rowl) dx = dx + defg[(b * p.S + s0) * NX + r];
        if (st) d.dX[(b * p.S + s0) * NX + r] = dx;
        lxx_row(p, wt.w(p, b), R.pc, r, R.lx);
        R.ru = rowl ? (real)(p.dt * r_diag(wt.w(p, b), r)) : (real)0;
        const bool stl = contact(R.pc, (rr % HC) / 3) != 0;
        R.cpl = rowl && (rr < HC ? stl : !stl);
        R.krow0 = (rr % HC) * NX;
        lin_row(p, R, r);
        out.ust = true;
        out.du = d.du + (b * p.Kc + k0) * NX + rr;
        out.dx = d.dX + (b * p.S + s0 + 1) * NX + rr;
        real q1s = 0, q2s = 0;
        for (int k = 0; k < N; k += 2) {
            lin_knot(p, S, B0, B1, k + 1 < N, k > 0, src, R, st, out, dx, q1s, q2s);
            if (k + 1 < N) lin_knot(p, S, B1, B0, k + 2 < N, true, src, R, st, out, dx, q1s, q2s);
        }
        lin_store_pending(true, st, out);
        const double *rec = d.term + (b * p.P + i) * TW;
        if (rowl) S.dx[hf][r] = dx;
        LSYNC();
        if (rowl) {
            q1s += (real)rec[TM_PHIX + r] * dx;
            real a = 0;
            for (int c = 0; c < NX; ++c) a += (real)rec[TM_PHIXX + r * NX + c] * S.dx[hf][c];
            q2s += dx * a;
        }
        v1 += half_sum(q1s);
        v2 += half_sum(q2s);
        LSYNC();
    }
#if HSDDP_STAMPS
    __syncthreads();
    if (lane < 8) d.dbg[(size_t)__builtin_amdgcn_readfirstlane((int)eb[1]) * 16 + 8 + lane] += lin_stamps().st[lane];
#endif
    if (r == 0 && act) merit_step(p, E, v1, v2);
}
void launch_lin_rollout(const Params &p, const Bufs &d, const Wts *weights, hipStream_t st)
{
    const dim3 g((unsigned)(p.elem_layout ? p.n_pairs : (p.B + 1) / 2));
    with_flags_table([&](auto f32, auto el, auto... wp) {
        using real = std::conditional_t<decltype(f32)::value, float, double>;
        hipLaunchKernelGGL((k_lin_rollout<real, decltype(el)::value>), g, dim3(64), 0, st, p, d, wp...);
    }, weights, p.fp32, p.elem_layout);
}

}
```

### hkd-mpc_amd/csrc/hsddp_lq.hip

```cpp
#include "hsddp_device.h"
#include "hsddp_dispatch.h"

namespace hsddp {

using namespace hkd;

#ifndef FWD_MINB
#define FWD_MINB 2
#endif

template <typename T> constexpr int LQ_STG = 128 / (int)sizeof(T) + 1;

template <typename T>
DEV void lq_flush(T *wl, const long *ridx, T *lq, int ldw, int lane, int OFF, int N)
{
    wave_sync();
    using T2 = std::conditional_t<std::is_same_v<T, float>, float2, double2>;
    const unsigned long long m = __ballot(1);
    const int na = __popcll(m), rank = __popcll(m & ((1ull << lane) - 1));
    for (int q = rank; q < 64 * (N / 2); q += na) {
        const int r = q / (N / 2), jp = q % (N / 2);
        const long rr = ridx[r];
        if (rr >= 0) {
            T2 w;
            w.x = wl[r * LQ_STG<T> + 2 * jp];
            w.y = wl[r * LQ_STG<T> + 2 * jp + 1];
            *reinterpret_cast<T2 *>(lq + rr * ldw + OFF + 2 * jp) = w;
        }
    }
    wave_sync();
}

#ifndef HSDDP_TERM_TPW
#define HSDDP_TERM_TPW 2
#endif
constexpr int TERM_TPW = HSDDP_TERM_TPW, TERM_TL = 64 / TERM_TPW;
struct TermLds {
    double sx[NX], shx[4][NX], scoef[4][2], sh[4], sxr[NX], spf[12], ssl[2 * MTD * 4];
    double sdw[NX + 12];
    double spx[12 * (NX + 1)];
    int sc[4], scn[4], smask[MTD];
};
static_assert(TERM_TL >= NX && TERM_TL >= 2 * MTD * 4 && TERM_TL >= 16, "terminal lane roles");

template <bool EL, typename TR>
DEV void terminal_task(const Params &p, const Bufs &d, const TR &terr, TermLds &S, int task, int t)
{
    const int b = task / p.P, i = task % p.P;
    const ElemState &E = d.el[b];
    if (E.done || E.inner_done) return;
    const auto L = layout_of<EL>(d, b);
    const int P = L.P();
    if (i >= P) return;
    double *sx = S.sx, (*shx)[NX] = S.shx, (*scoef)[2] = S.scoef, *sh = S.sh, *sxr = S.sxr, *spf = S.spf, *ssl = S.ssl;
    int *sc = S.sc, *scn = S.scn, *smask = S.smask;
    const int s = L.s0(i) + L.N(i);
    const double *xr = ref_ptr(p, d.ref_x, b, s, NX), *pf = ref_ptr(p, d.ref_foot, b, s, 12);
    if (t < NX) {
        sx[t] = xbuf(d, work_buf(d, b))[((size_t)b * p.S + s) * NX + t];
        sxr[t] = xr[t];
    }
    if (t < 2 * MTD * 4) ssl[t] = (t < MTD * 4 ? d.al_sigma : d.al_lambda)[((size_t)b * p.P + i) * MTD * 4 + (t & (MTD * 4 - 1))];
    constexpr int MK = TERM_TL - MTD;
    if (t >= MK) smask[t - MK] = d.td_mask[((size_t)b * p.P + i) * MTD + t - MK];
    if (t >= 4 && t < 16) spf[t - 4] = pf[t - 4];
    if (t < 4) {
        const int *cc = d.contacts + ((size_t)b * (p.P + 1) + i) * 4;
        sc[t] = cc[t]; scn[t] = cc[4 + t];
    }
    wave_sync();
    double *spx = S.spx;
    const bool bnd = i < P - 1;
    for (int e = t; e < 4 * NX; e += TERM_TL) (&shx[0][0])[e] = 0.0;
    if (bnd)
        for (int e = t; e < 12 * (NX + 1); e += TERM_TL) spx[e] = (e / (NX + 1) + 12 == e % (NX + 1)) ? 1.0 : 0.0;
    double *strig = S.sdw;
    unsigned need = td_union(smask);
#pragma unroll
    for (int l = 0; l < 4; ++l) need |= (bnd && touchdown(sc, scn, l)) ? 1u << l : 0u;
    if (need && t < 15) {
        const int m = t - 3;
        const double a = t < 3 ? sx[t] : m % 3 == 2 ? sx[11 + m] + sx[12 + m] : sx[12 + m];
        sincos(a, &strig[2 * t], &strig[2 * t + 1]);
    }
    wave_sync();
    if (t < 4) {
        const int l = t;
        const bool tdc = (td_union(smask) >> l) & 1, tdr = touchdown(sc, scn, l);
        double h = 0.0;
        if (tdc || (bnd && tdr)) {
            Rot R, Dy, Dp, Dr;
            const EulTrig tr{strig[1], strig[0], strig[3], strig[2], strig[5], strig[4]};
            rot_zyx(tr, R);
            rot_zyx_grad(tr, Dy, Dp, Dr);
            double pb[3], dpb[3][3];
            foot_body_trig(l, strig + 6 + 6 * l, pb, dpb);
            shx[l][0] = Dy.r[2][0] * pb[0] + Dy.r[2][1] * pb[1] + Dy.r[2][2] * pb[2];
            shx[l][1] = Dp.r[2][0] * pb[0] + Dp.r[2][1] * pb[1] + Dp.r[2][2] * pb[2];
            shx[l][2] = Dr.r[2][0] * pb[0] + Dr.r[2][1] * pb[1] + Dr.r[2][2] * pb[2];
#pragma unroll
            for (int k = 0; k < 3; ++k) shx[l][12 + 3 * l + k] = R.r[2][0] * dpb[0][k] + R.r[2][1] * dpb[1][k] + R.r[2][2] * dpb[2][k];
            shx[l][5] = 1.0;
            h = (sx[5] + R.r[2][0] * pb[0] + R.r[2][1] * pb[1] + R.r[2][2] * pb[2]) - terr.ground(p, b, i);
            if (!tdc) {
                h = 0.0;
#pragma unroll
                for (int j = 0; j < NX; ++j) shx[l][j] = 0.0;
            }
            if (bnd && tdr) {
#pragma unroll
                for (int k = 0; k < 3; ++k) {
                    double *row = spx + (3 * l + k) * (NX + 1);
                    row[12 + 3 * l + k] = 0.0;
                    if (k == 2) continue;
                    row[0] = Dy.r[k][0] * pb[0] + Dy.r[k][1] * pb[1] + Dy.r[k][2] * pb[2];
                    row[1] = Dp.r[k][0] * pb[0] + Dp.r[k][1] * pb[1] + Dp.r[k][2] * pb[2];
                    row[2] = Dr.r[k][0] * pb[0] + Dr.r[k][1] * pb[1] + Dr.r[k][2] * pb[2];
                    row[3 + k] = 1.0;
#pragma unroll
                    for (int m = 0; m < 3; ++m)
                        row[12 + 3 * l + m] = R.r[k][0] * dpb[0][m] + R.r[k][1] * dpb[1][m] + R.r[k][2] * dpb[2][m];
                }
            }
        } else if (bnd && sc[l] && !scn[l]) {
#pragma unroll
            for (int k = 0; k < 3; ++k) spx[(3 * l + k) * (NX + 2) + 12] = 0.0;
        }
        double c0 = 0.0, c1 = 0.0;
        if (tdc && p.AL_active)
            for (int q = 0; q < MTD; ++q)
                if ((smask[q] >> l) & 1) {
                    const double sg = ssl[4 * q + l], lm = ssl[MTD * 4 + 4 * q + l];
                    const double hq = (smask[q] & TD_STALE) ? 0.0 : h;
                    c0 += sg * hq + lm;
                    c1 += sg * (1 + hq) + lm;
                }
        scoef[l][0] = c0;
        scoef[l][1] = c1;
        sh[l] = h;
    }
    wave_sync();
    const auto &w = terr.w(p, b);
    const auto &kp = terr.wk(b);
    double *rec = d.term + ((size_t)b * p.P + i) * TW;
    if (t == 0) {
        double tv;
        d.slot_cost[(size_t)b * p.S + s] = terminal_cost_h(p, w, sc, sx, sxr, spf, smask, ssl, ssl + MTD * 4, sh, tv);
    }
    if (t < NX) {
        const int j = t;
        double v = kp.qf_gain * kp.qf_scale[j] * q_diag(kp, sc, j) * (sx[j] - sxr[j]);
        if (j >= 3 && j < 6) {
            for (int l = 0; l < 4; ++l) {
                int m = 3 * l + (j - 3);
                double e = (sx[12 + m] - sx[j]) - (spf[m] - sxr[j]);
                v += -(w.foot_term_grad * sc[l] * foot_weight(kp, sc, m) * e);
            }
        } else if (j >= 12) {
            int m = j - 12, l = m / 3;
            double e = (sx[j] - sx[3 + m % 3]) - (spf[m] - sxr[3 + m % 3]);
            v += w.foot_term_grad * sc[l] * foot_weight(kp, sc, m) * e;
        }
        for (int l = 0; l < 4; ++l) v += scoef[l][0] * shx[l][j];
        rec[TM_PHIX + j] = v;
    }
    auto fw = [&](int l, int j) { return w.foot_term_grad * sc[l] * sc[l] * foot_weight(kp, sc, 3 * l + j); };
    double *sdd = S.sdw, *scw = S.sdw + NX;
    if (t < NX) {
        const int r = t;
        double v = kp.qf_gain * kp.qf_scale[r] * q_diag(kp, sc, r);
        if (r >= 3 && r < 6) {
            for (int l = 0; l < 4; ++l) v += fw(l, r - 3);
        } else if (r >= 12) {
            v += fw((r - 12) / 3, (r - 12) % 3);
        }
        sdd[r] = v;
    }
    if (t < 12) scw[t] = fw(t / 3, t % 3);
    wave_sync();
    bool use[4];
#pragma unroll
    for (int l = 0; l < 4; ++l) use[l] = scoef[l][1] != 0.0;
    int r = t / NX, cidx = t % NX;
    for (int e = t; e < NN; e += TERM_TL) {
        double v = 0.0;
        if (r == cidx)
            v = sdd[r];
        else if (r >= 3 && r < 6 && cidx >= 12 && (cidx - 12) % 3 == r - 3)
            v = -scw[cidx - 12];
        else if (cidx >= 3 && cidx < 6 && r >= 12 && (r - 12) % 3 == cidx - 3)
            v = -scw[r - 12];
#pragma unroll
        for (int l = 0; l < 4; ++l)
            if (use[l]) v += scoef[l][1] * (shx[l][r] * shx[l][cidx]);
        rec[TM_PHIXX + e] = v;
        if (bnd && r >= 12) rec[TM_PX + e] = spx[(r - 12) * (NX + 1) + cidx];
        r += TERM_TL / NX;
        cidx += TERM_TL % NX;
        if (cidx >= NX) {
            cidx -= NX;
            r += 1;
        }
    }
}

template <typename WT>
DEV void lq_lu_reb(const Params &p, const WT &w, double mu, const int *c, const double *u, const double *ovr, const double *ur, const double *dl,
                   const double *ep, double *lu, double *rb)
{
#pragma unroll
    for (int j = 0; j < NU; ++j) lu[j] = p.dt * r_diag(w, j) * (u[j] - ur[j]);
#pragma unroll
    for (int j = 0; j < 24; ++j) rb[j] = 0.0;
    auto reb = [&](auto uniform) {
        constexpr bool U = decltype(uniform)::value;
        const double inv_du = p.grf_inv_delta;
#pragma unroll
        for (int lg = 0; lg < 4; ++lg) {
            if (!c[lg]) continue;
            double gu[3] = {0, 0, 0}, hu[6] = {0, 0, 0, 0, 0, 0};
            const double f0 = grf_force(u, ovr, 3 * lg), f1 = grf_force(u, ovr, 3 * lg + 1), f2 = grf_force(u, ovr, 3 * lg + 2);
#pragma unroll
            for (int r = 0; r < 5; ++r) {
                double row[3], d1, d2;
                grf_row(mu, r, row);
                double g = row[0] * f0 + row[1] * f1 + row[2] * f2;
                const double dlr = U ? p.grf_delta : dl[5 * lg + r];
                reb_derivs(g, dlr, U ? inv_du : 1.0 / dlr, d1, d2);
                double e = U ? p.grf_eps : ep[5 * lg + r];
                for (int a = 0; a < 3; ++a) gu[a] += e * d1 * row[a];
                hu[0] += e * (d2 * row[0] * row[0]); hu[1] += e * (d2 * row[0] * row[1]);
                hu[2] += e * (d2 * row[0] * row[2]); hu[3] += e * (d2 * row[1] * row[1]);
                hu[4] += e * (d2 * row[1] * row[2]); hu[5] += e * (d2 * row[2] * row[2]);
            }
            for (int a = 0; a < 3; ++a) lu[3 * lg + a] += p.dt * gu[a];
            for (int a = 0; a < 6; ++a) rb[6 * lg + a] = p.dt * hu[a];
        }
    };
    if (p.ReB_active) {
        if (p.reb_uniform) reb(std::true_type{});
        else reb(std::false_type{});
    }
}

template <bool EL, typename TR>
DEV void terminal_wave(const Params &p, const Bufs &d, const TR &terr, TermLds *S, long wave, int lane)
{
    if (p.retry_cap > 0 && wave == 0 && lane == 0) *d.retry_count = 0;
    if (wave == 0)
        for (int t = lane; t < LS_LIVE; t += 64) d.ls_live[t] = 0;
    if (wave == 0 && lane < 4) d.counter[lane] = 0;
    const int h = lane / TERM_TL;
    const long task = wave * TERM_TPW + h;
    if (task < (long)p.B * p.P) terminal_task<EL>(p, d, terr, S[h], (int)task, lane % TERM_TL);
}

template <bool F32, bool EL, bool SLOTS, typename... TR>
__global__ __launch_bounds__(256, FWD_MINB) void k_lq(Params p, Bufs d, TR... tr)
{
    const auto terr = terrain_of(tr...);
    using T = std::conditional_t<F32, float, double>;
    constexpr size_t STG = sizeof(T) * 4 * 64 * LQ_STG<T>, TRM = 4 * TERM_TPW * sizeof(TermLds);
    __shared__ __attribute__((aligned(16))) char lds[STG > TRM ? STG : TRM];
    T (*stage)[64 * LQ_STG<T>] = reinterpret_cast<T (*)[64 * LQ_STG<T>]>(lds);
    __shared__ long sridx[4][64];
    const int lane = threadIdx.x & 63, w = threadIdx.x >> 6;
    constexpr bool BY_KNOT = !SLOTS && !F32;
    const long nunit = (long)p.B * (BY_KNOT ? p.Kc : p.S);
    const long nknot = (nunit + 255) / 256;
    if ((long)blockIdx.x >= nknot) {
        terminal_wave<EL>(p, d, terr, reinterpret_cast<TermLds *>(lds) + w * TERM_TPW, ((long)blockIdx.x - nknot) * 4 + w, lane);
        return;
    }
    sridx[w][lane] = -1;
    const long gid = (long)blockIdx.x * blockDim.x + threadIdx.x;
    if (gid >= nunit) return;
    const int b = (int)(gid / (BY_KNOT ? p.Kc : p.S));
    const ElemState &E = d.el[b];
    if (E.done || E.inner_done) return;
    const auto L = layout_of<EL>(d, b);
    int i, k, s;
    if constexpr (BY_KNOT) {
        const int kc0 = (int)(gid % p.Kc);
        knot_phase(L, kc0, i, k);
        if (k >= L.N(i)) return;
        s = L.s0(i) + k;
    } else {
        s = (int)(gid % p.S);
        if (s >= L.S()) return;
        slot_phase(L, s, i, k);
    }
    int c[4], cn[4];
    load_contacts(d, p, b, i, c, cn);
    double x[NX];
    const int wb = work_buf(d, b);
    const double *xg = xbuf(d, wb) + ((size_t)b * p.S + s) * NX;
#pragma unroll
    for (int j = 0; j < NX; ++j) x[j] = xg[j];
    const double *dg = dbuf(d, wb) + ((size_t)b * p.S + s) * NX;
    if (SLOTS) {
        double fs = 0.0;
#pragma unroll
        for (int j = 0; j < NX; ++j) fs += dg[j] * dg[j];
        d.slot_feas[(size_t)b * p.S + s] = fs;
    }
    if constexpr (F32) {
        float *d32 = d.def32 + ((size_t)b * p.S + s) * NX;
#pragma unroll
        for (int j = 0; j < NX; ++j) d32[j] = (float)dg[j];
    }
    const double *xr = ref_ptr(p, d.ref_x, b, s, NX), *pf = ref_ptr(p, d.ref_foot, b, s, 12);
    if (k == L.N(i)) return;
    const int kc = L.k0(i) + k;
    sridx[w][lane] = (long)b * p.Kc + kc;
    double u[NU];
    const double *ug = ubuf(d, wb) + ((size_t)b * p.Kc + kc) * NU;
#pragma unroll
    for (int j = 0; j < NU; ++j) u[j] = ug[j];
    const double *ovr = constraint_forces(d, E, b, kc);
    const double *ur = ref_ptr(p, d.ref_u, b, s, NU);
    const double *dl = d.reb_delta + ((size_t)b * p.Kc + kc) * 20, *ep = d.reb_eps + ((size_t)b * p.Kc + kc) * 20;
    const double mu = terr.mu(p, b, i);
    const auto &wr = terr.w(p, b);
    if (SLOTS) {
        double viol;
        d.slot_cost[(size_t)b * p.S + s] = running_cost(p, wr, mu, c, x, u, xr, ur, pf, dl, ep, viol, ovr);
    }

    T *lqT = F32 ? (T *)d.lq32 : (T *)d.lq;
    const int ldw = F32 ? LQW32 : LQW;
    double cd[4] = {(double)c[0], (double)c[1], (double)c[2], (double)c[3]};
    T *wl = stage[w];
    constexpr int W = 128 / (int)sizeof(T);
    auto col = [&](int pos) -> T & { return wl[lane * LQ_STG<T> + (pos & (W - 1))]; };
    auto put = [&](int pos, double v) {
        col(pos) = (T)v;
        if ((pos & (W - 1)) == W - 1) lq_flush(wl, sridx[w], lqT, ldw, lane, pos - (W - 1), W);
    };
    col(15) = 0;
    hkd_partial_emit(x, u, cd, p.dt, [&](int piece, int j, double v) {
        const int pos = piece == 0 ? LQ_SE + j : piece == 1 ? sw_at(j / 17, j % 17) : bw_at(j / 12, j % 12);
        col(pos) = (T)v;
        if (pos < 96 && ((pos & (W - 1)) == W - 1 || (W == 16 && pos == 14))) {
            lq_flush(wl, sridx[w], lqT, ldw, lane, pos & ~(W - 1), W);
            if (pos == 63) col(67) = 0;
        }
    });
    {
        double lx[NX];
#pragma unroll
        for (int j = 0; j < NX; ++j) lx[j] = p.dt * q_diag(wr, c, j) * (x[j] - xr[j]);
#pragma unroll
        for (int j = 0; j < 12; ++j) {
            double e = (x[12 + j] - x[3 + j % 3]) - (pf[j] - xr[3 + j % 3]);
            double v = p.dt * c[j / 3] * foot_weight(wr, c, j) * e;
            lx[3 + j % 3] += -v;
            lx[12 + j] += v;
        }
#pragma unroll
        for (int j = 0; j < NX; ++j) put(LQ_LX + j, lx[j]);
    }
    double lu[NU], rb[24];
    lq_lu_reb(p, wr, mu, c, u, ovr, ur, dl, ep, lu, rb);
#pragma unroll
    for (int j = 0; j < NU; ++j) put(LQ_LU + j, lu[j]);
#pragma unroll
    for (int j = 0; j < 24; ++j) put(LQ_RB + j, rb[j]);
    if constexpr (F32)
#pragma unroll
        for (int j = LQW; j < LQW32; ++j) put(j, 0.0);
}

template <bool EL, typename... TR>
__global__ __launch_bounds__(128, 4) void k_terminal(Params p, Bufs d, TR... tr)
{
    __shared__ TermLds S[2 * TERM_TPW];
    const int w = threadIdx.x >> 6;
    terminal_wave<EL>(p, d, terrain_of(tr...), S + w * TERM_TPW, (long)blockIdx.x * 2 + w, threadIdx.x & 63);
}

void launch_lq(const Params &p, const Bufs &d, const double *terrain, const Wts *weights, hipStream_t st)
{
    const unsigned nterm = blocks_for((long)p.B * p.P, 4 * TERM_TPW);
    const bool merged = nterm <= 256;
    const bool by_knot = !p.lq_slots && !p.fp32;
    if (!merged) {
        const unsigned nt2 = blocks_for((long)p.B * p.P, 2 * TERM_TPW);
        with_flags_tables([&](auto el, auto... tr) {
            hipLaunchKernelGGL(k_terminal<decltype(el)::value>, dim3(nt2), dim3(128), 0, st, p, d, tr...);
        }, terrain, weights, p.elem_layout);
    }
    const dim3 g(blocks_for((long)p.B * (by_knot ? p.Kc : p.S), 256) + (merged ? nterm : 0));
    with_flags_tables([&](auto f32, auto el, auto slots, auto... tr) {
        hipLaunchKernelGGL((k_lq<decltype(f32)::value, decltype(el)::value, decltype(slots)::value>), g, dim3(256), 0, st, p, d,
                           tr...);
    }, terrain, weights, p.fp32, p.elem_layout, p.lq_slots);
}

}
```

### hkd-mpc_amd/csrc/hsddp_solve.cpp

```cpp
#include <cstdlib>
#include <cstring>
#include <utility>

#include "hsddp_handle.h"

using namespace hsddp;

namespace {
struct Timer {
    hipStream_t st;
    bool on;
    std::vector<hipEvent_t> *pool;
    size_t used = 0;
    std::vector<std::pair<hipEvent_t, hipEvent_t>> ev[5];
    hipEvent_t pend = nullptr;
    hipEvent_t next()
    {
        if (used == pool->size()) {
            hipEvent_t e;
            hipEventCreate(&e);
            pool->push_back(e);
        }
        return (*pool)[used++];
    }
    void begin(int cat, hipEvent_t &e0)
    {
        if (!on) return;
        (void)cat;
        if (pend) {
            e0 = pend;
            pend = nullptr;
            return;
        }
        e0 = next();
        hipEventRecord(e0, st);
    }
    void cut() { pend = nullptr; }
    void end(int cat, hipEvent_t e0)
    {
        if (!on) return;
        hipEvent_t e1 = next();
        hipEventRecord(e1, st);
        ev[cat].push_back({e0, e1});
        pend = e1;
    }
    double total(int cat)
    {
        double t = 0;
        for (auto &pr : ev[cat]) {
            float ms = 0;
            hipEventElapsedTime(&ms, pr.first, pr.second);
            t += ms;
        }
        ev[cat].clear();
        return t;
    }
};
}

static int count_active(hsddp_handle h, int which, int &n)
{
    HIPCHK(hipMemsetAsync(h->d.counter, 0, 4 * sizeof(int), h->stream));
    launch_count(h->p, h->d, which, h->stream);
    HIPCHK(hipMemcpyAsync(h->host_counter, h->d.counter, 4 * sizeof(int), hipMemcpyDeviceToHost, h->stream));
    HIPCHK(hipStreamSynchronize(h->stream));
    n = h->host_counter[which];
    return HSDDP_OK;
}

static int solve_check(hsddp_handle h)
{
    if (!h) return fail(HSDDP_ERR_ARG, "null handle");
    if (!h->have_problem) return fail(HSDDP_ERR_ARG, "upload the problem first");
    if (h->need_inputs) return fail(HSDDP_ERR_ARG, "the layout changed (hsddp_shift): call hsddp_update_problem first");
    HIPCHK(hipSetDevice(h->desc.device));
    h->sim_fresh = false;
    if (int rc = sync_terrain(h)) return rc;
    return sync_weights(h);
}

static std::vector<double> ls_steps(double alpha)
{
    std::vector<double> trials;
    for (double eps = 1; eps > 1e-3; eps *= alpha) trials.push_back(eps);
    return trials;
}

static void sync_ref_columns(hsddp_handle h)
{
    if (!h->ref_cols_stale) return;
    launch_ref_columns(h->p, h->d, h->Bref, h->stream);
    h->ref_cols_stale = false;
}

static void begin_launches(hsddp_handle h)
{
    if (h->p.trace) hipMemsetAsync(h->d.dbg, 0, (size_t)h->p.B * 16 * sizeof(unsigned long long), h->stream);
    sync_ref_columns(h);
    launch_reset_elements(h->p, h->d, h->stream);
    launch_rollout(h->p, h->d, 0.0, 0, 1, -1, budget_of(h), terrain_of(h), weights_of(h), h->stream);
    launch_decide(h->p, h->d, 0.0, 0, 1, -1, budget_of(h), terrain_of(h), weights_of(h), h->stream);
    h->slots_fresh = true;
}

static void iteration_launches(hsddp_handle h, const std::vector<double> &trials, Timer &tm)
{
    const Params &p = h->p;
    const Bufs &d = h->d;
    hipStream_t st = h->stream;
    hipEvent_t e0;
    tm.begin(0, e0);
    {
        Params pl = p;
        pl.lq_slots = h->slots_fresh ? 0 : 1;
        launch_lq(pl, d, terrain_of(h), weights_of(h), st);
    }
    tm.end(0, e0);
    tm.begin(1, e0);
    launch_riccati(p, d, weights_of(h), st);
    tm.end(1, e0);
    if (!p.ms0) {
        tm.begin(4, e0);
        launch_lin_rollout(p, d, weights_of(h), st);
        tm.end(4, e0);
    }
    tm.begin(2, e0);
    for (size_t t = 0; t < trials.size(); ++t) {
        launch_rollout(p, d, trials[t], t + 1 == trials.size(), 0, (int)t, budget_of(h), terrain_of(h), weights_of(h), st);
        launch_decide(p, d, trials[t], t + 1 == trials.size(), 0, (int)t, budget_of(h), terrain_of(h), weights_of(h), st);
    }
    tm.end(2, e0);
    h->slots_fresh = true;
}

static bool graphs_enabled()
{
    const char *e = std::getenv("HSDDP_NO_GRAPH");
    return !(e && *e && *e != '0');
}

static int graph_launch(hsddp_handle h, const std::vector<double> &trials, int par)
{
    Params pl = h->p;
    pl.lq_slots = h->slots_fresh ? 0 : 1;
    hsddp_handle_t::IterGraph *hit = nullptr;
    for (auto &c : h->iter_graph)
        if (c.exec && c.par == par && !std::memcmp(&c.p, &pl, sizeof(Params)) &&
            !std::memcmp(&c.d, &h->d, sizeof(Bufs)) && c.alpha == h->opt.alpha && c.budget == budget_of(h) &&
            c.terrain == terrain_of(h) && c.weights == weights_of(h))
            hit = &c;
    if (!hit) {
        auto &g = h->iter_graph[h->iter_graph_next];
        h->iter_graph_next = (h->iter_graph_next + 1) % 8;
        if (g.exec) {
            HIPCHK(hipStreamSynchronize(h->stream));
            HIPCHK(hipGraphExecDestroy(g.exec));
        }
        g.exec = nullptr;
        HIPCHK(hipStreamBeginCapture(h->stream, hipStreamCaptureModeThreadLocal));
        Timer off{h->stream, false, &h->events};
        iteration_launches(h, trials, off);
        launch_count(h->p, h->d, 1, h->stream);
        hipError_t e = hipMemcpyAsync(h->host_counter + 8 + 4 * par, h->d.counter, 4 * sizeof(int), hipMemcpyDeviceToHost,
                               h->stream);
        hipGraph_t graph = nullptr;
        const hipError_t ec = hipStreamEndCapture(h->stream, &graph);
        if (e == hipSuccess) e = ec;
        if (e == hipSuccess) e = hipGraphInstantiate(&g.exec, graph, nullptr, nullptr, 0);
        if (graph) hipGraphDestroy(graph);
        if (e != hipSuccess) {
            g.exec = nullptr;
            return fail(HSDDP_ERR_DEVICE, std::string("iteration graph: ") + hipGetErrorString(e));
        }
        std::memcpy(&g.p, &pl, sizeof(Params));
        std::memcpy(&g.d, &h->d, sizeof(Bufs));
        g.alpha = h->opt.alpha;
        g.budget = budget_of(h);
        g.terrain = terrain_of(h);
        g.weights = weights_of(h);
        g.par = par;
        hit = &g;
    }
    if (!h->iter_done[par]) HIPCHK(hipEventCreateWithFlags(&h->iter_done[par], hipEventDisableTiming));
    HIPCHK(hipGraphLaunch(hit->exec, h->stream));
    HIPCHK(hipEventRecord(h->iter_done[par], h->stream));
    h->slots_fresh = true;
    return HSDDP_OK;
}

static int graph_wait(hsddp_handle h, int par, int &n_active)
{
    HIPCHK(hipEventSynchronize(h->iter_done[par]));
    n_active = h->host_counter[8 + 4 * par + 1];
    return HSDDP_OK;
}

static void outer_end_launches(hsddp_handle h, Timer &tm)
{
    hipEvent_t e0;
    tm.begin(3, e0);
    if (h->opt.ReB_active && !h->p.reb_uniform) {
        h->slots_fresh = false;
        h->reb_at_init = false;
    }
    if (h->opt.ReB_active) launch_reb_update(h->p, h->d, terrain_of(h), h->stream);
    launch_outer_end(h->p, h->d, budget_of(h), h->stream);
    tm.end(3, e0);
}

static int finish_stats(hsddp_handle h, Timer &tm, hipEvent_t e0, hsddp_stats *stats, int iters, int outers, int nbwd)
{
    HIPCHK(hipGetLastError());
    HIPCHK(hipStreamSynchronize(h->stream));
    if (!stats) return HSDDP_OK;
    hipEvent_t e1;
    hipEventCreate(&e1);
    hipEventRecord(e1, h->stream);
    hipEventSynchronize(e1);
    float ms = 0;
    hipEventElapsedTime(&ms, e0, e1);
    hipEventDestroy(e0);
    hipEventDestroy(e1);
    stats->ms_total = ms;
    stats->ms_lq = tm.total(0);
    stats->ms_backward = tm.total(1);
    stats->ms_forward = tm.total(2);
    stats->ms_other = tm.total(3);
    stats->ms_linear = tm.total(4);
    stats->inner_iterations = iters;
    stats->outer_iterations = outers;
    stats->n_backward_launches = nbwd;
    HIPCHK(hipMemsetAsync(h->d.counter + 4, 0, 2 * sizeof(int), h->stream));
    launch_stat_sums(h->p, h->d, h->stream);
    HIPCHK(hipMemcpyAsync(h->host_counter + 4, h->d.counter + 4, 2 * sizeof(int), hipMemcpyDeviceToHost, h->stream));
    HIPCHK(hipStreamSynchronize(h->stream));
    stats->ls_trials = h->host_counter[4];
    stats->element_iterations = h->host_counter[5];
    return HSDDP_OK;
}

static hipEvent_t start_stats(hsddp_handle h, hsddp_stats *stats)
{
    if (!stats) return nullptr;
    memset(stats, 0, sizeof(*stats));
    hipEvent_t e0;
    hipEventCreate(&e0);
    hipEventRecord(e0, h->stream);
    return e0;
}

extern "C" int hsddp_solve(hsddp_handle h, hsddp_stats *stats)
{
    int rc = solve_check(h);
    if (rc) return rc;
    Timer tm{h->stream, stats != nullptr, &h->events};
    hipEvent_t e0 = start_stats(h, stats);
    const std::vector<double> trials = ls_steps(h->opt.alpha);
    begin_launches(h);
    int iters = 0, outers = 0, nbwd = 0;
    const bool checks = !h->opt.no_early_exit;
    const bool graph = checks && graphs_enabled();
    const int n_outer = outer_bound(h), n_inner = inner_bound(h);
    for (int ou = 0; ou < n_outer; ++ou) {
        tm.cut();
        launch_outer_begin(h->p, h->d, budget_of(h), h->stream);
        outers++;
        for (int in = 0; in < n_inner; ++in) {
            if (graph) {
                int n = 0;
                tm.cut();
                if (in == 0 && (rc = graph_launch(h, trials, 0))) return rc;
                if (in + 1 < n_inner && (rc = graph_launch(h, trials, (in + 1) & 1))) return rc;
                if ((rc = graph_wait(h, in & 1, n))) return rc;
                iters++;
                nbwd++;
                if (n == 0) break;
                continue;
            }
            iteration_launches(h, trials, tm);
            iters++;
            nbwd++;
            if (checks) {
                int n = 0;
                tm.cut();
                if ((rc = count_active(h, 1, n))) return rc;
                if (n == 0) break;
            }
        }
        outer_end_launches(h, tm);
        if (checks) {
            int n = 0;
            tm.cut();
            if ((rc = count_active(h, 2, n))) return rc;
            if (n == 0) break;
        }
    }
    return finish_stats(h, tm, e0, stats, iters, outers, nbwd);
}

extern "C" int hsddp_solve_begin(hsddp_handle h)
{
    int rc = solve_check(h);
    if (rc) return rc;
    begin_launches(h);
    launch_outer_begin(h->p, h->d, budget_of(h), h->stream);
    HIPCHK(hipGetLastError());
    return HSDDP_OK;
}

extern "C" int hsddp_iterate(hsddp_handle h, int n, hsddp_stats *stats)
{
    int rc = solve_check(h);
    if (rc) return rc;
    if (n < 0) return fail(HSDDP_ERR_ARG, "negative iteration count");
    Timer tm{h->stream, stats != nullptr, &h->events};
    hipEvent_t e0 = start_stats(h, stats);
    const std::vector<double> trials = ls_steps(h->opt.alpha);
    sync_ref_columns(h);
    for (int i = 0; i < n; ++i) iteration_launches(h, trials, tm);
    return finish_stats(h, tm, e0, stats, n, 0, n);
}

extern "C" int hsddp_solve_end(hsddp_handle h)
{
    int rc = solve_check(h);
    if (rc) return rc;
    Timer tm{h->stream, false, &h->events};
    outer_end_launches(h, tm);
    HIPCHK(hipGetLastError());
    HIPCHK(hipStreamSynchronize(h->stream));
    return HSDDP_OK;
}
```

### hkd-mpc_amd/csrc/hsddp_sweep.hip

```cpp
#include "hsddp_wave.h"
#include "hsddp_dispatch.h"

namespace hsddp {

using namespace hkd;

namespace sweep {

#ifndef HSDDP_STAMPS
#define HSDDP_STAMPS 0
#endif
#ifndef SWEEP_WPB2_WPE
#define SWEEP_WPB2_WPE 1
#endif
#if HSDDP_STAMPS
#define STAMP(n)                                                                              \
    do {                                                                                      \
        __builtin_amdgcn_sched_barrier(0);                                                    \
        unsigned long long t_;                                                                \
        asm volatile("s_waitcnt lgkmcnt(0)\n\ts_memtime %0\n\ts_waitcnt lgkmcnt(0)" : "=s"(t_)::"memory"); \
        __builtin_amdgcn_sched_barrier(0);                                                    \
        if (threadIdx.x == 0) {                                                               \
            if ((n) > 0) S.st[n] += t_ - S.tprev;                                             \
            S.tprev = t_;                                                                     \
        }                                                                                     \
    } while (0)
#else
#define STAMP(n) \
    do {         \
    } while (0)
#endif

constexpr int PRIO_DENSE = 0, PRIO_MIXED = 1, PRIO_CHAIN = 2;
#define PRIO(level) __builtin_amdgcn_s_setprio(level)

#define SSYNC()                              \
    do {                                     \
        asm volatile("" ::: "memory");       \
        __builtin_amdgcn_sched_barrier(0);   \
    } while (0)

#define CSYNC()                                              \
    do {                                                     \
        asm volatile("s_waitcnt lgkmcnt(0)" ::: "memory");   \
        __builtin_amdgcn_s_barrier();                        \
        asm volatile("" ::: "memory");                       \
        __builtin_amdgcn_sched_barrier(0);                   \
    } while (0)

constexpr int HC = 12;
constexpr int MS = 26;
constexpr int TS = 14;
constexpr int WS = 25;
constexpr int V_SE = LQ_SE, V_D = 104, V_LX = 128, V_LU = 152, V_RB = 176, VW = 200;
static_assert(LQ_BW + 36 == V_D && LQ_LX + 24 == V_LX && LQ_LU + 24 == V_LU && LQ_RB + 24 == V_RB, "image layout");

template <typename real>
struct alignas(16) Lds {
    real img[2][VW];
    real zero[32];
    struct alignas(16) Item {
        real TI[24 * TS];
        real MI[25 * MS];
        real du[24];
        real pc[8];
    } it[2];
#if HSDDP_STAMPS
    unsigned long long st[12], tprev;
#endif
};
static_assert(sizeof(Lds<double>) <= 20480, "two waves per SIMD on 160 KB of LDS need <= 20 KB per wave");

template <typename real>
struct alignas(16) LdsCS {
    real img[2][2][VW];
    real zero[32];
    struct alignas(16) Item {
        real TI[24 * TS];
        real MZ[2][25 * MS];
        real du[24];
        real pc[8];
    } it[2];
    int fl[2];
};
static_assert(sizeof(LdsCS<double>) <= 40960, "four split workgroups per CU on 160 KB of LDS need <= 40 KB each");

template <typename real>
struct Pieces {
    static constexpr int E = 16 / sizeof(real);
    static constexpr int NA = V_D / E, ND = NX / E, NR = (LQW - V_D) / E, NP = NA + ND + NR;
    static constexpr int NI = (2 * NP + 63) / 64;
    static_assert(NP * E == VW && V_D % E == 0, "16-byte pieces");
};

template <typename real> struct Prec;
template <> struct Prec<double> {
    static DEV const double *lq(const Bufs &d) { return d.lq; }
    static DEV double *K(const Bufs &d) { return d.K; }
    static DEV const double *def(const Bufs &d, int b) { return kdbuf(work_buf(d, b)); }
    static constexpr int LQS = LQW;
};
template <> struct Prec<float> {
    static DEV const float *lq(const Bufs &d) { return d.lq32; }
    static DEV float *K(const Bufs &d) { return d.K32; }
    static DEV const float *def(const Bufs &d, int) { return d.def32; }
    static constexpr int LQS = LQW32;
};

template <typename T>
using Global = __attribute__((address_space(1))) T *;

template <typename real>
struct Item {
    int b;
    bool act;
    real reg;
    Global<real> K;
    Global<double> dU;
};

template <typename real>
struct Phase {
    int cmask;
    int xmask;
    real lxd;
    real xw;
    real dtr;
    real dtrz;
};


template <typename real, typename ItemT, typename WT>
DEV void load_phase(const Params &p, const Bufs &d, ItemT &I, int b, int i, int pp, Phase<real> &ph, const WT &wt)
{
    const auto &ww = wt.w(p, b);
    const auto &wk = wt.wk(b);
    const int *cs = d.contacts + ((size_t)b * (p.P + 1) + i) * 4;
    int c[4];
#pragma unroll
    for (int l = 0; l < 4; ++l) c[l] = cs[l];
    ph.cmask = 0;
#pragma unroll
    for (int l = 0; l < 4; ++l) ph.cmask |= (c[l] != 0) << l;
    SSYNC();
    if (pp < 8) {
        const int cl = (ph.cmask >> (pp & 3)) & 1;
        I.pc[pp] = pp < 4 ? (cl ? (real)p.dt_m : (real)0) : (cl ? (real)0 : (real)p.dt);
    }
    SSYNC();
    const int pos = pp & 15, cq = (ph.cmask >> ((pos / 3) & 3)) & 1;
    ph.dtr = (real)(p.dt * (cq ? ww.r_grf : ww.r_qJd));
    const int cz = (ph.cmask >> ((pp < HC ? pp : 0) / 3)) & 1;
    ph.dtrz = (real)(p.dt * (cz ? ww.r_qJd : ww.r_grf));
    const int r = pp < NX ? pp : 0;
    double dg = p.dt * (r < 12 ? wk.qbase[r] : ww.q_qJ * (1 - ((ph.cmask >> ((r - 12) / 3)) & 1)));
    ph.xmask = 0;
    ph.xw = 0;
    if (r >= 3 && r < 6) {
        const double fw = p.dt * (ww.foot_gain * wk.foot_w[r - 3]);
#pragma unroll
        for (int l = 0; l < 4; ++l) dg += c[l] ? fw : 0.0;
        ph.xmask = ph.cmask;
        ph.xw = (real)fw;
    } else if (r >= 12) {
        const int m = r - 12;
        const double w = ((ph.cmask >> (m / 3)) & 1) ? p.dt * (ww.foot_gain * wk.foot_w[m % 3]) : 0.0;
        dg += w;
        ph.xmask = 1;
        ph.xw = (real)w;
    }
    ph.lxd = (real)dg;
}

template <typename real>
DEV void fetch(Lds<real> &S, const real *rec0, const real *def0, const real *rec1, const real *def1, int lane)
{
    using PC = Pieces<real>;
    asm volatile("s_waitcnt lgkmcnt(0)" ::: "memory");
#pragma unroll
    for (int t = 0; t < PC::NI; ++t) {
        const int n = 64 * t + lane;
        if (n < 2 * PC::NP) {
            const int e = n >= PC::NP, q = n - e * PC::NP;
            const real *rec = e ? rec1 : rec0, *def = e ? def1 : def0;
            const real *src = q < PC::NA ? rec + PC::E * q : q < PC::NA + PC::ND ? def + PC::E * (q - PC::NA)
                                                                                 : rec + PC::E * (q - PC::ND);
            lds_dma16(src, (unsigned)(size_t)(&S.img[0][0]) + 1024u * t);
        }
    }
}

template <int W, typename real>
DEV void fetch_cs(LdsCS<real> &S, int q, const real *rec0, const real *def0, const real *rec1, const real *def1,
                  int lane)
{
    using PC = Pieces<real>;
    constexpr int H = (PC::NI + 1) / 2;
#pragma unroll
    for (int u = 0; u < H; ++u) {
        const int t = W * H + u;
        const int n = 64 * t + lane;
        if (t < PC::NI && n < 2 * PC::NP) {
            const int e = n >= PC::NP, qq = n - e * PC::NP;
            const real *rec = e ? rec1 : rec0, *def = e ? def1 : def0;
            const real *src = qq < PC::NA ? rec + PC::E * qq : qq < PC::NA + PC::ND ? def + PC::E * (qq - PC::NA)
                                                                                    : rec + PC::E * (qq - PC::ND);
            lds_dma16(src, (unsigned)(size_t)(&S.img[q][0][0]) + 1024u * t);
        }
    }
}

DEV constexpr int rb_index(int a, int b)
{
    return (a < b ? a : b) == 0 ? (a > b ? a : b) : (a < b ? a : b) == 1 ? 2 + (a > b ? a : b) : 5;
}

struct Lane {
    int lane, e, pp, pos;
    bool row;
    bool qlane;
    int rb[3];
    int xc0, xkind;
};
DEV Lane make_lane();

constexpr unsigned CS_COLS1 = (1u << 0) | (1u << 3) | (1u << 4) | (1u << 5) | (1u << 8) | (1u << 9) | (1u << 10) |
                              (1u << 11) | (1u << 18) | (1u << 19) | (1u << 21) | (1u << 22);
DEV constexpr int cs_wave(int c) { return (int)((CS_COLS1 >> c) & 1u); }
template <int W>
DEV constexpr bool cs_mine(int c) { return W < 0 || cs_wave(c) == W; }

template <int MASK>
DEV constexpr bool stance(int l) { return MASK < 0 || ((MASK >> l) & 1); }
template <int MASK>
DEV constexpr bool swing(int l) { return MASK < 0 || !((MASK >> l) & 1); }
template <int MASK>
DEV constexpr bool sw_live(int q) { return q < 9 || stance<MASK>((q - 9) >> 1); }

template <int W = -1, int MASK = -1, typename real>
DEV void emit_SA(real (&acc)[NX], const real (&x)[NX], const real (&cf)[8], real dt)
{
    auto sw_row = [&](auto I) {
        constexpr int i = I;
        static_for<17>([&](auto Q) {
            if constexpr (cs_mine<W>(sw_col(Q)) && sw_live<MASK>(Q)) vfma<sw_at(i, Q)>(acc[sw_col(Q)], cf, x[6 + i]);
        });
    };
    auto se_row = [&](auto I) {
        constexpr int i = I;
        static_for<5>([&](auto Q) {
            if constexpr (cs_mine<W>(se_col(Q))) vfma<V_SE + 5 * i + Q>(acc[se_col(Q)], cf, x[i]);
        });
    };
    sw_row(std::integral_constant<int, 0>{});
    se_row(std::integral_constant<int, 0>{});
    sw_row(std::integral_constant<int, 1>{});
    se_row(std::integral_constant<int, 1>{});
    sw_row(std::integral_constant<int, 2>{});
    se_row(std::integral_constant<int, 2>{});
    static_for<3>([&](auto A) {
        if constexpr (cs_mine<W>(9 + A)) acc[9 + A] = __builtin_fma(x[3 + A], dt, acc[9 + A]);
    });
}

template <int Q0 = 0, int Q1 = HC, int MASK = -1, typename real>
DEV void emit_Bc(real (&acc)[HC], real y6, real y7, real y8, const real *y9, const real *y12, const real (&bv)[4],
                 const real (&bq)[4], const real (&cf)[8])
{
#pragma unroll
    for (int q = Q0; q < Q1; ++q)
        if (swing<MASK>(q / 3)) acc[q] = __builtin_fma(y12[q], bq[q / 3], acc[q]);
#pragma unroll
    for (int q = Q0; q < Q1; ++q)
        if (stance<MASK>(q / 3)) acc[q] = __builtin_fma(y9[q % 3], bv[q / 3], acc[q]);
    static_for<Q1 - Q0>([&](auto Q) {
        if constexpr (stance<MASK>((Q0 + Q) / 3)) vfma<bw_at(0, Q0 + Q)>(acc[Q0 + Q], cf, y6);
    });
    static_for<Q1 - Q0>([&](auto Q) {
        if constexpr (stance<MASK>((Q0 + Q) / 3)) vfma<bw_at(1, Q0 + Q)>(acc[Q0 + Q], cf, y7);
    });
    static_for<Q1 - Q0>([&](auto Q) {
        if constexpr (stance<MASK>((Q0 + Q) / 3)) vfma<bw_at(2, Q0 + Q)>(acc[Q0 + Q], cf, y8);
    });
}

template <typename real>
DEV void eliminate(real (&w)[HC], real (&w2)[HC], unsigned long long &bad)
{
    constexpr bool F64 = sizeof(real) == 8;
    constexpr int CH = F64 ? 13 : 9;
    real r, e, nf, nf2;
    {
        const real piv = row_bcast<0>(w[0]);
        bad |= __builtin_amdgcn_ballot_w64(!(piv > (real)1e-9));
        asm_rcp(r, piv);
        asm_nfma1(e, piv, r);
        asm_newton(r, e);
        if constexpr (F64) {
            asm_nfma1(e, piv, r);
            asm_newton(r, e);
        }
        asm_nmul(nf, w[0], r);
        asm_nmul(nf2, w2[0], r);
    }
    static_for<HC>([&](auto J) {
        constexpr int j = J, jn = j + 1;
        constexpr bool nx = jn < HC;
        real pivn = 0, rn = 0, en = 0, nfn = 0, nf2n = 0;
        if constexpr (nx) {
            bfma<j>(w2[jn], w[jn], nf2);
            fmac_row_bcast<j, false>(w[jn], nf);
        }
        constexpr int NO = nx ? HC - 2 - j : 0;
        constexpr int NT = (2 * NO > CH + 1) ? 2 * NO : CH + 1;
        static_for<NT>([&](auto T) {
            constexpr int t = T, i = jn + 1 + t / 2;
            if constexpr (t < 2 * NO) {
                if constexpr (t % 2 == 0)
                    bfma<j>(w2[i], w[i], nf2);
                else
                    fmac_row_bcast<j, false>(w[i], nf);
            }
            if constexpr (nx) {
                if constexpr (t == 1) pivn = row_bcast<(nx ? jn : 0)>(w[jn]);
                if constexpr (t == 3) asm_rcp(rn, pivn);
                if constexpr (t == 5) asm_nfma1(en, pivn, rn);
                if constexpr (t == 7) asm_newton(rn, en);
                if constexpr (F64 && t == 9) asm_nfma1(en, pivn, rn);
                if constexpr (F64 && t == 11) asm_newton(rn, en);
                if constexpr (t == CH) {
                    asm_nmul(nfn, w[jn], rn);
                    asm_nmul(nf2n, w2[jn], rn);
                }
            }
        });
        w[j] = nf;
        w2[j] = nf2;
        if constexpr (nx) {
            bad |= __builtin_amdgcn_ballot_w64(!(pivn > (real)1e-9));
            nf = nfn;
            nf2 = nf2n;
        }
    });
    static_for<HC - 1>([&](auto Jr) {
        constexpr int j = HC - 1 - Jr;
        static_for<j>([&](auto Ii) {
            constexpr int i = j - 1 - Ii;
            bfma<j>(w2[i], w[i], w2[j]);
        });
    });
}

template <int W, bool DV, int MASK = -1, typename real, typename LdsT>
DEV void knot(real dt, LdsT &S, const Lane &L, const Phase<real> &ph, const Item<real> &it, int kc,
              real (&h)[NX], real &g, bool &live, bool first, bool more, int ib, int par, const real *nrec0,
              const real *ndef0, const real *nrec1, const real *ndef1, double &dvs)
{
    constexpr bool CS = W >= 0;
    constexpr int Q0 = CS ? 6 * W : 0, Q1 = CS ? Q0 + 6 : HC;
    auto &I = S.it[L.e];
    const real *img;
    real *ma = nullptr, *za = nullptr;
    if constexpr (CS) {
        img = S.img[ib][L.e];
        ma = I.MZ[par];
        za = I.MZ[par ^ 1];
    } else {
        img = S.img[L.e];
    }
    auto MA = [&]() -> real * { if constexpr (CS) return ma; else return I.MI; };
    auto ZA = [&]() -> real * { if constexpr (CS) return za; else return I.MI; };
    const int pp = L.pp, pos = L.pos;
    const real reg = it.reg;
    const int cmask = MASK >= 0 ? MASK : ph.cmask;
    if constexpr (!CS) STAMP(0);
    if constexpr (!CS) PRIO(PRIO_CHAIN);
    if (first) {
        asm volatile("s_waitcnt vmcnt(0)" ::: "memory");
        if constexpr (CS) CSYNC();
    }
    real cf[8];
#pragma unroll
    for (int k = 0; k < 8; ++k) cf[k] = img[16 * k + pos];
    real bv[4], bq[4];
#pragma unroll
    for (int l = 0; l < 4; ++l) { bv[l] = I.pc[l]; bq[l] = I.pc[4 + l]; }
    if constexpr (!CS) STAMP(1);
    if constexpr (!CS) PRIO(PRIO_DENSE);
    real t[HC], ga[4] = {g, 0, 0, 0};
#pragma unroll
    for (int q = 0; q < HC; ++q) t[q] = 0;
    emit_Bc<Q0, Q1, MASK>(t, h[6], h[7], h[8], h + 9, h + 12, bv, bq, cf);
    static_for<NX>([&](auto C) { vfma<V_D + C>(ga[C & 3], cf, h[C]); });
    const real gn = (ga[0] + ga[1]) + (ga[2] + ga[3]);
    pin(t);
    real h9[NX];
#pragma unroll
    for (int j = 0; j < 9; ++j) h9[j] = h[j];
#pragma unroll
    for (int j = 9; j < NX; ++j) h9[j] = 0;
    SSYNC();
    real (&m)[NX] = h;
    emit_SA<W, MASK>(m, h9, cf, dt);
    pin(t);
    pin(m);
    if (L.row) {
        static_for<NX>([&](auto C) {
            if constexpr (cs_mine<W>(C)) MA()[pp * MS + C] = m[C];
        });
        if constexpr (W <= 0) MA()[pp * MS + NX] = gn;
#pragma unroll
        for (int q = Q0; q < Q1; ++q) I.TI[pp * TS + q] = t[q];
    }
    if constexpr (CS) CSYNC(); else SSYNC();
    if constexpr (!CS) STAMP(2);
    if constexpr (!CS) PRIO(PRIO_MIXED);
    const int pc = pp < MS - 1 ? pp : MS - 1;
    real mc[NX];
#pragma unroll
    for (int j = 0; j < NX; ++j) mc[j] = MA()[j * MS + pc];
    real w2[HC];
#pragma unroll
    for (int l = 0; l < 4; ++l) {
        const real *lcp = pp == NX ? img + V_LU + (((cmask >> l) & 1) ? 3 * l : 12 + 3 * l) : S.zero;
#pragma unroll
        for (int a = 0; a < 3; ++a) w2[3 * l + a] = lcp[a];
    }
    emit_SA<W, MASK>(m, mc, cf, dt);
    emit_Bc<0, HC, MASK>(w2, mc[6], mc[7], mc[8], mc + 9, mc + 12, bv, bq, cf);
    pin(m);
    pin(w2);
    if constexpr (!CS) STAMP(3);
    if constexpr (!CS) PRIO(PRIO_CHAIN);
    if (pp <= NX) {
#pragma unroll
// ... 271 lines not shown
                if constexpr (sizeof(real) == 4) dpp_ready(px);
                static_for<8>([&](auto Kk) {
                    static_for<NX>([&](auto Cc) { vfma<NX * Kk + Cc>(wr[Cc], px, h[8 * Kc + Kk]); });
                });
            });
            SSYNC();
            if (L.row) {
#pragma unroll
                for (int c = 0; c < NX; ++c) WI[pp * WS + c] = wr[c];
                WI[pp * WS + NX] = g;
            }
            SSYNC();
            const int pc = pp < NX ? pp : NX;
            real wc[NX];
#pragma unroll
            for (int j = 0; j < NX; ++j) wc[j] = WI[j * WS + pc];
            real vr[NX];
#pragma unroll
            for (int c = 0; c < NX; ++c) vr[c] = 0;
            static_for<3>([&](auto Kc) {
                real px[12];
#pragma unroll
                for (int k = 0; k < 12; ++k) px[k] = (real)Px[192 * Kc + 16 * k + L.pos];
                if constexpr (sizeof(real) == 4) dpp_ready(px);
                static_for<8>([&](auto Jj) {
                    static_for<NX>([&](auto Cc) { vfma<NX * Jj + Cc>(vr[Cc], px, wc[8 * Kc + Jj]); });
                });
            });
            SSYNC();
            if (pp == NX)
#pragma unroll
                for (int c = 0; c < NX; ++c) WI[NX * WS + c] = vr[c];
            SSYNC();
            const real gp = WI[NX * WS + (L.row ? pp : 0)];
#pragma unroll
            for (int c = 0; c < NX; ++c) h[c] = L.row ? (real)rec[TM_PHIXX + pp * NX + c] + vr[c] : (real)0;
            g = L.row ? (real)rec[TM_PHIX + pp] + gp : (real)0;
            SSYNC();
            if constexpr (CS) CSYNC();
        }
        const int N = PL.N(i), s0 = PL.s0(i), k0 = PL.k0(i);
        const real *rec0 = lqg + ((size_t)b0 * p.Kc + k0) * Prec<real>::LQS, *def0 = defg0 + ((size_t)b0 * p.S + s0 + 1) * NX;
        const real *rec1 = lqg + ((size_t)b1 * p.Kc + k0) * Prec<real>::LQS, *def1 = defg1 + ((size_t)b1 * p.S + s0 + 1) * NX;
        if constexpr (CS || DV) {
            phase_knots<-1, CSW, DV>((real)p.dt, S, L, ph, it, N, k0, rec0, def0, rec1, def1, h, g, live, fail, dvs, ib, par);
        } else {
            real *row = S.it[L.e].MI + pp * MS;
            if (L.row) {
#pragma unroll
                for (int c = 0; c < NX; ++c) row[c] = h[c];
                row[NX] = g;
            }
            SSYNC();
            const int m0 = __builtin_amdgcn_readlane(ph.cmask, 0), m1 = __builtin_amdgcn_readlane(ph.cmask, 32);
            const bool both = masks && m0 == m1 && __builtin_amdgcn_ballot_w64(live) == ~0ull;
            const int flags = ph.cmask | (ph.xmask << 4);
            PhaseOut o{dvs, live, fail};
#define HSDDP_PHASE(MASK)                                                                                              \
    phase_knots_masked<MASK, DV, WPE, real>((unsigned)(size_t)&S, flags, ph.lxd, ph.xw, ph.dtr, ph.dtrz, it.reg, it.K, \
                                            it.dU, (real)p.dt, N, k0, rec0, def0, rec1, def1, &o)
            if (both && m0 == MASK_TROT_A) HSDDP_PHASE(MASK_TROT_A);
            else if (both && m0 == MASK_TROT_B) HSDDP_PHASE(MASK_TROT_B);
            else HSDDP_PHASE(-1);
#undef HSDDP_PHASE
            dvs = o.dvs; live = o.live != 0; fail = o.fail;
#pragma unroll
            for (int c = 0; c < NX; ++c) h[c] = L.row ? row[c] : (real)0;
            g = L.row ? row[NX] : (real)0;
            SSYNC();
        }
        asm volatile("s_waitcnt vmcnt(0)" ::: "memory");
        if (!__builtin_amdgcn_ballot_w64(live)) break;
        const real *d0 = (L.e ? defg1 : defg0) + ((size_t)b * p.S + s0) * NX;
        real dc[2] = {d0[L.pos], L.pos < NX - 16 ? d0[16 + L.pos] : (real)0};
        real a = 0;
        static_for<NX>([&](auto Cc) { vfma<Cc>(a, dc, h[Cc]); });
        if (L.row) g += a;
        if (p.store_value && live && L.row && CSW <= 0) {
            double *V = d.value0 + ((size_t)b * p.P + i) * (NX + NN);
#pragma unroll
            for (int c = 0; c < NX; ++c) V[NX + pp * NX + c] = (double)h[c];
            V[pp] = (double)g;
        }
    }
    if constexpr (DV) {
#pragma unroll
        for (int o = 16; o > 0; o >>= 1) dvs += __shfl_xor(dvs, o);
    }
    dv = dvs;
    return it.act ? fail : -1;
}

constexpr int STAGE_SLOTS = 512;

template <typename ItemT>
DEV double *cost_stage(const Params &p, ItemT &item)
{
    const bool fits = p.S <= STAGE_SLOTS && 2 * (size_t)p.S * sizeof(double) <= sizeof(ItemT);
    return fits ? reinterpret_cast<double *>(&item) : nullptr;
}

template <bool EL>
DEV void element_cost(const Params &p, const Bufs &d, int b, int lane, double *stg, double &cost, double &feas)
{
    const auto LY = layout_of<EL>(d, b);
    const int P = LY.P(), g = lane & 31;
    const double *c = d.slot_cost + (size_t)b * p.S, *f = d.slot_feas + (size_t)b * p.S;
    if (stg) {
        const int Sel = LY.S();
#pragma unroll
        for (int t = 0; t < STAGE_SLOTS / 32; ++t) {
            const int sl = g + 32 * t;
            if (sl < Sel) {
                stg[sl] = c[sl];
                stg[p.S + sl] = f[sl];
            }
        }
        __builtin_amdgcn_fence(__ATOMIC_RELEASE, "wavefront");
        __builtin_amdgcn_wave_barrier();
        __builtin_amdgcn_fence(__ATOMIC_ACQUIRE, "wavefront");
        c = stg;
        f = stg + p.S;
    }
    double ci = 0.0, fi = 0.0;
    if (g < P) {
        const int N = LY.N(g), s0 = LY.s0(g);
#pragma unroll 10
        for (int k = 0; k < N; ++k) {
            ci += c[s0 + k];
            fi += f[s0 + k];
        }
        ci += c[s0 + N];
        fi += f[s0 + N];
    }
    cost = 0.0; feas = 0.0;
    for (int i = 0; i < P; ++i) {
        cost += __shfl(ci, (lane & 32) + i);
        feas += __shfl(fi, (lane & 32) + i);
    }
    feas = sqrt(feas);
}

DEV Lane make_lane()
{
    Lane L;
    L.lane = threadIdx.x & 63;
    L.e = L.lane >> 5;
    L.pp = L.lane & 31;
    L.pos = L.lane & 15;
    L.row = L.pp < NX;
    L.qlane = L.pos < HC;
    const int lq = (L.qlane ? L.pos : 0) / 3, aq = L.pos % 3;
#pragma unroll
    for (int a = 0; a < 3; ++a) L.rb[a] = V_RB + 6 * lq + rb_index(aq, a);
    L.xkind = (L.pp >= 3 && L.pp < 6) ? 1 : (L.pp >= 12 && L.pp < NX) ? 2 : 0;
    L.xc0 = L.xkind == 1 ? 12 + (L.pp - 3) : L.xkind == 2 ? 3 + (L.pp - 12) % 3 : MS - 1;
    return L;
}

template <typename LdsT>
DEV void zero_init(LdsT &S, int lane)
{
    if (lane < 32) S.zero[lane] = 0;
    SSYNC();
}

template <bool EL, typename Idx>
DEV void pair_element(const Params &p, const Bufs &d, const Lane &L, Idx pair, int &bv, bool &valid)
{
    int b;
    if constexpr (EL) {
        const int e0 = d.pairs[2 * pair], e1 = d.pairs[2 * pair + 1];
        b = L.e ? e1 : e0;
        valid = b >= 0;
        bv = valid ? b : (L.e ? e0 : e1);
    } else {
        b = 2 * pair + L.e;
        valid = b < p.B;
        bv = valid ? b : p.B - 1;
    }
}

}

using namespace sweep;

template <typename real, bool EL, bool DV, int WPB, typename... WP>
__global__ __launch_bounds__(64 * WPB) __attribute__((amdgpu_waves_per_eu(WPB == 2 ? SWEEP_WPB2_WPE : 2))) void k_riccati(Params p, Bufs d, int masks, WP... wp)
{
    const auto wt = terrain_of(wp...);
    __shared__ Lds<real> SS[WPB];
    const int wv = WPB > 1 ? __builtin_amdgcn_readfirstlane((int)(threadIdx.x >> 6)) : 0;
    Lds<real> &S = SS[wv];
    const int pair = (int)blockIdx.x * WPB + wv;
    const Lane L = make_lane();
    zero_init(S, L.lane);
#if HSDDP_STAMPS
    if (L.lane < 12) S.st[L.lane] = 0;
#endif
    if constexpr (EL)
        if (pair >= p.n_pairs) return;
    int bv;
    bool valid;
    pair_element<EL>(p, d, L, pair, bv, valid);
    ElemState &E = d.el[bv];
    bool act = valid && !E.done && !E.inner_done;
    if (!__builtin_amdgcn_ballot_w64(act)) return;
    double ecost, efeas;
    {
        double *stg = cost_stage(p, S.it[L.e]);
        element_cost<EL>(p, d, bv, L.lane, stg, ecost, efeas);
        SSYNC();
    }
    double reg = E.reg;
    Item<real> it;
    it.b = bv;
    it.K = (Global<real>)(Prec<real>::K(d) + (size_t)bv * p.Kc * KCW);
    it.dU = (Global<double>)(d.dU + (size_t)bv * p.Kc * NX);
    bool need = act, ok = false;
    double dvk = 0.0;
    for (int attempt = 0; __builtin_amdgcn_ballot_w64(need); ++attempt) {
        it.act = need;
        it.reg = (real)reg;
        double dv;
        const int fk = sweep_pair<real, EL, DV, -1, (WPB == 2 ? SWEEP_WPB2_WPE : 2)>(p, d, S, L, it, dv, masks != 0, wt);
        if (need) {
            if (fk < 0) {
                ok = true;
                need = false;
                dvk = dv;
            } else {
                bool deferred = false;
                if (attempt == 0 && p.retry_cap > 0) {
                    int f = 0;
                    if (L.pp == 0) {
                        f = atomicAdd(d.retry_count, 1);
                        if (f < p.retry_cap) d.retry_list[f] = RetryEntry{bv, 0, reg};
                    }
                    f = __shfl(f, L.lane & 32);
                    deferred = f < p.retry_cap;
                }
                if (deferred) {
                    need = false;
                    if (L.pp == 0) { E.iters += 1; E.cost = ecost; E.feas = efeas; E.accepted = 0; }
                    act = false;
                } else {
                    reg = fmax(reg * p.update_regularization, 1e-03);
                    if (reg > 1e2 || attempt >= MAX_REG_ATTEMPTS) need = false;
                }
            }
        }
    }
#if HSDDP_STAMPS
    SSYNC();
    if (L.lane < 12) d.dbg[(size_t)__builtin_amdgcn_readfirstlane(bv) * 16 + L.lane] += S.st[L.lane];
#endif
    if (act && L.pp == 0) {
        double rn = reg / 20;
        if (rn < 1e-06) rn = 0;
        E.iters += 1; E.cost = ecost; E.feas = efeas; E.accepted = 0;
        if (ok) E.reg = rn;
        else { E.reg = rn; E.status = 1; E.done = 1; E.ls_active = 0; }
        if (DV && ok) merit_step(p, E, dvk, -dvk);
    }
}
template <bool EL, bool DV, int W, typename WT>
DEV void riccati_cs_wave(const Params &p, const Bufs &d, LdsCS<double> &S, const WT &wt)
{
    using real = double;
    const Lane L = make_lane();
    int bv;
    bool valid;
    pair_element<EL>(p, d, L, blockIdx.x, bv, valid);
    ElemState &E = d.el[bv];
    bool act = valid && !E.done && !E.inner_done;
    if (!__builtin_amdgcn_ballot_w64(act)) return;
    double ecost = 0, efeas = 0;
    if (W == 0) {
        double *stg = cost_stage(p, S.it[L.e]);
        element_cost<EL>(p, d, bv, L.lane, stg, ecost, efeas);
    }
    CSYNC();
    double reg = E.reg;
    Item<real> it;
    it.b = bv;
    it.K = (Global<real>)(d.K + (size_t)bv * p.Kc * KCW);
    it.dU = (Global<double>)(d.dU + (size_t)bv * p.Kc * NX);
    bool need = act, ok = false;
    double dvk = 0.0;
    for (int attempt = 0; __builtin_amdgcn_ballot_w64(need); ++attempt) {
        it.act = need;
        it.reg = (real)reg;
        double dv;
        const int fk = sweep_pair<real, EL, DV, W>(p, d, S, L, it, dv, false, wt);
        if (attempt == 0 && p.retry_cap > 0) {
            if (W == 0 && need && fk >= 0 && L.pp == 0) {
                const int f = atomicAdd(d.retry_count, 1);
                if (f < p.retry_cap) d.retry_list[f] = RetryEntry{bv, 0, reg};
                S.fl[L.e] = f;
            }
            CSYNC();
        }
        if (need) {
            if (fk < 0) {
                ok = true;
                need = false;
                dvk = dv;
// ... 197 lines not shown
```

Before: 1.193 million.

## Regroup LQ record into per-leg-pair blocks and skip writing/loading swing-leg blocks

Reorders the per-knot LQ record so the coefficients belonging to each pair of legs sit in whole-cache-line blocks. Blocks whose legs are all in swing are no longer written by the LQ kernel or DMA'd by the linear rollout; they are pre-zeroed once and zero-filled in LDS instead. This targets memory traffic in the bandwidth-bound LQ and linear-rollout stages. The cost is considerably more complex index mapping, extra setup launches and per-lane skip masks, and correctness depends on the pre-zeroed blocks staying valid.

Result: no change. 1.203 million, median of 6 (+0.8%).

```diff
diff --git a/hkd-mpc_amd/csrc/hkd_model.h b/hkd-mpc_amd/csrc/hkd_model.h
--- a/hkd-mpc_amd/csrc/hkd_model.h
+++ b/hkd-mpc_amd/csrc/hkd_model.h
@@ -272,7 +272,8 @@
         }
     }
 #pragma unroll
-    for (int l = 0; l < 4; ++l)
+    for (int n = 0; n < 4; ++n) {
+        const int l = n == 0 ? 0 : n == 1 ? 3 : n == 2 ? 1 : 2;
 #pragma unroll
         for (int k = 0; k < 2; ++k) {
             double v[3];
@@ -280,8 +281,6 @@
             for (int i = 0; i < 3; ++i) v[i] = -tl(l, i, k);
             col(v, 9 + 2 * l + k);
         }
-#pragma unroll
-    for (int l = 0; l < 4; ++l) {
         double r0 = x[12 + 3 * l] - x[3], r1 = x[13 + 3 * l] - x[4], r2 = -x[5];
         double Sr[3][3] = {{0.0, -r2, r1}, {r2, 0.0, -r0}, {-r1, r0, 0.0}};
 #pragma unroll
@@ -292,6 +291,7 @@
             inertia_inv_apply(v, o);
             emit(2, 3 * l + k, dt * o[0]); emit(2, 12 + 3 * l + k, dt * o[1]); emit(2, 24 + 3 * l + k, dt * o[2]);
         }
+        if (n & 1) emit(3, n >> 1, 0.0);
     }
 }
 
diff --git a/hkd-mpc_amd/csrc/hsddp_api.cpp b/hkd-mpc_amd/csrc/hsddp_api.cpp
--- a/hkd-mpc_amd/csrc/hsddp_api.cpp
+++ b/hkd-mpc_amd/csrc/hsddp_api.cpp
@@ -35,6 +35,8 @@
     {
         const char *tr = std::getenv("HSDDP_TRACE");
         p.trace = (tr && tr[0] == '1') ? 1 : 0;
+        const char *sk = std::getenv("HSDDP_LQ_SKIP");
+        p.lq_skip = (sk && sk[0] == '0') ? 0 : 1;
     }
     p.mu = ds.cparams.mu_fric;
     p.grf_delta = ds.cparams.grf_delta; p.grf_delta_min = ds.cparams.grf_delta_min; p.grf_eps = ds.cparams.grf_eps;
@@ -1189,21 +1191,27 @@
             const int i = phase_of_control(layout_of(h, b), (int)kc);
             const int *c = h->contacts.data() + (b * (p.P + 1) + i) * 4;
             const size_t o = (b * Kc + kc);
+            const int cmask = (c[0] != 0) | (c[1] != 0) << 1 | (c[2] != 0) << 2 | (c[3] != 0) << 3;
+            auto at = [&](int pos) {
+                if (p.fp32) return r[lq_pos32(pos)];
+                if (p.lq_skip && pos >= LQ_BLK && pos < LQ_LX && lq_block_skipped(cmask, (pos - LQ_BLK) / LQ_BLKW)) return 0.0;
+                return r[pos];
+            };
             if (A) {
                 double *a = A + o * NN;
                 std::fill(a, a + NN, 0.0);
                 for (int j = 0; j < NX; ++j) a[j * NX + j] = 1.0;
                 for (int rr = 0; rr < 3; ++rr)
-                    for (int q = 0; q < 5; ++q) a[rr * NX + hkd::se_col(q)] += r[LQ_SE + 5 * rr + q];
+                    for (int q = 0; q < 5; ++q) a[rr * NX + hkd::se_col(q)] += at(LQ_SE + 5 * rr + q);
                 for (int q = 0; q < 3; ++q) a[(3 + q) * NX + 9 + q] += dt;
                 for (int rr = 0; rr < 3; ++rr)
-                    for (int q = 0; q < 17; ++q) a[(6 + rr) * NX + hkd::sw_col(q)] += r[sw_at(rr, q)];
+                    for (int q = 0; q < 17; ++q) a[(6 + rr) * NX + hkd::sw_col(q)] += at(sw_at(rr, q));
             }
             if (Bm) {
                 double *bb = Bm + o * NN;
                 std::fill(bb, bb + NN, 0.0);
                 for (int rr = 0; rr < 3; ++rr)
-                    for (int q = 0; q < 12; ++q) bb[(6 + rr) * NX + q] = r[bw_at(rr, q)];
+                    for (int q = 0; q < 12; ++q) bb[(6 + rr) * NX + q] = at(bw_at(rr, q));
                 for (int lg = 0; lg < 4; ++lg)
                     for (int a = 0; a < 3; ++a) {
                         bb[(9 + a) * NX + 3 * lg + a] = dt * c[lg] / hkd::kMass;
@@ -1213,8 +1221,8 @@
             Wts wr;
             weights_row(weights_of(h, b), wr);
             if (l) l[o] = cost[b * S + kc + i];
-            if (lx) for (int j = 0; j < NX; ++j) lx[o * NX + j] = r[LQ_LX + j];
-            if (lu) for (int j = 0; j < NX; ++j) lu[o * NX + j] = r[LQ_LU + j];
+            if (lx) for (int j = 0; j < NX; ++j) lx[o * NX + j] = at(LQ_LX + j);
+            if (lu) for (int j = 0; j < NX; ++j) lu[o * NX + j] = at(LQ_LU + j);
             if (lxx) {
                 double *m = lxx + o * NN;
                 std::fill(m, m + NN, 0.0);
@@ -1235,7 +1243,7 @@
                 static const int ix[3][3] = {{0, 1, 2}, {1, 3, 4}, {2, 4, 5}};
                 for (int lg = 0; lg < 4; ++lg)
                     for (int a = 0; a < 3; ++a)
-                        for (int e = 0; e < 3; ++e) m[(3 * lg + a) * NX + 3 * lg + e] += r[LQ_RB + 6 * lg + ix[a][e]];
+                        for (int e = 0; e < 3; ++e) m[(3 * lg + a) * NX + 3 * lg + e] += at(rb_at(lg, ix[a][e]));
             }
         }
     return HSDDP_OK;
diff --git a/hkd-mpc_amd/csrc/hsddp_internal.h b/hkd-mpc_amd/csrc/hsddp_internal.h
--- a/hkd-mpc_amd/csrc/hsddp_internal.h
+++ b/hkd-mpc_amd/csrc/hsddp_internal.h
@@ -4,6 +4,7 @@
 #include <cstddef>
 #include "hkd_model.h"
 #include "hsddp_phases.h"
+#include "hsddp_lq_layout.h"
 
 namespace hsddp {
 
@@ -14,18 +15,6 @@
 constexpr int TD_PENDING = 0x10;
 constexpr int KCW = 12 * 24;
 
-constexpr int LQ_SE = 0;
-constexpr int LQ_SW = 16;
-constexpr int LQ_BW = 68;
-constexpr int LQ_LX = 104;
-constexpr int LQ_LU = 128;
-constexpr int LQ_RB = 152;
-constexpr int LQW = 176;
-constexpr int LQW32 = 192;
-constexpr int sw_at(int r, int q) { return LQ_SW + 3 * q + r; }
-constexpr int bw_at(int r, int k) { return LQ_BW + 3 * k + r; }
-static_assert(LQ_SE + 15 < LQ_SW && LQ_SW + 51 < LQ_BW && LQ_BW + 36 == LQ_LX && LQ_LX + 24 == LQ_LU &&
-              LQ_LU + 24 == LQ_RB && LQ_RB + 24 == LQW, "record layout");
 
 constexpr int MAX_REG_ATTEMPTS = 64;
 
@@ -58,6 +47,7 @@
     int store_value;
     int ms0;
     int trace;
+    int lq_skip;
 };
 
 struct Wts {
@@ -122,6 +112,7 @@
 
 
 void launch_lq(const Params &p, const Bufs &d, const double *terrain, const Wts *weights, hipStream_t st);
+void launch_lq_zero_blocks(const Params &p, const Bufs &d, hipStream_t st);
 
 void launch_riccati(const Params &p, const Bufs &d, const Wts *weights, hipStream_t st);
 void launch_lin_rollout(const Params &p, const Bufs &d, const Wts *weights, hipStream_t st);
diff --git a/hkd-mpc_amd/csrc/hsddp_linear.hip b/hkd-mpc_amd/csrc/hsddp_linear.hip
--- a/hkd-mpc_amd/csrc/hsddp_linear.hip
+++ b/hkd-mpc_amd/csrc/hsddp_linear.hip
@@ -38,13 +38,13 @@
 
 template <typename real> struct Prec;
 template <> struct Prec<double> {
-    static constexpr int LQS = LQW;
+    static constexpr int LQS = LQW, LQI = LIN_LQW;
     static DEV const double *lq(const Bufs &d) { return d.lq; }
     static DEV double *K(const Bufs &d) { return d.K; }
     static DEV const double *def(const Bufs &d, int b) { return kdbuf(work_buf(d, b)); }
 };
 template <> struct Prec<float> {
-    static constexpr int LQS = LQW32;
+    static constexpr int LQS = LQW32, LQI = LQW32;
     static DEV const float *lq(const Bufs &d) { return d.lq32; }
     static DEV float *K(const Bufs &d) { return d.K32; }
     static DEV const float *def(const Bufs &d, int) { return d.def32; }
@@ -59,14 +59,17 @@
 };
 
 template <typename real>
-DEV void load_phase(const Params &p, const Bufs &d, const size_t (&b)[2], int hf, int i, PhaseConst<real> &pc)
+DEV void load_phase(const Params &p, const Bufs &d, const size_t (&b)[2], int hf, int i, PhaseConst<real> &pc, int (&cm)[2])
 {
     typedef const __attribute__((address_space(4))) int cint;
     cint *c0 = (cint *)(d.contacts + (b[0] * (p.P + 1) + i) * 4), *c1 = (cint *)(d.contacts + (b[1] * (p.P + 1) + i) * 4);
     pc.cmask = 0;
+    cm[0] = cm[1] = 0;
 #pragma unroll
     for (int l = 0; l < 4; ++l) {
         const int a0 = c0[l], a1 = c1[l];
+        cm[0] |= (a0 != 0) << l;
+        cm[1] |= (a1 != 0) << l;
         pc.c[l] = hf ? a1 : a0;
         pc.cmask |= (pc.c[l] != 0) << l;
         pc.bv[l] = pc.c[l] ? (real)p.dt_m : (real)0;
@@ -134,13 +137,14 @@
 
 template <typename real>
 struct LinImg {
-    static constexpr int K = 0;
-    static constexpr int LQ = K + KCW * (int)sizeof(real);
-    static constexpr int D = LQ + Prec<real>::LQS * (int)sizeof(real);
+    static constexpr int LQ = 0;
+    static constexpr int K = LQ + Prec<real>::LQI * (int)sizeof(real);
+    static constexpr int D = K + KCW * (int)sizeof(real);
     static constexpr int DU = D + NX * (int)sizeof(real);
     static constexpr int END = DU + NX * 8;
     static constexpr int NI = (END / 16 + 63) / 64;
-    static_assert(LQ % 16 == 0 && D % 16 == 0 && DU % 16 == 0 && END % 16 == 0 && (NI == 4 || NI == 3), "16-byte pieces");
+    static_assert(K % 16 == 0 && D % 16 == 0 && DU % 16 == 0 && END % 16 == 0 && (NI == 4 || NI == 3), "16-byte pieces");
+    static_assert(sizeof(real) == 4 || (LQ + (LQ_CEND + 2 * LQ_BLK_END) * 8 <= 1024), "the pair blocks in the first instruction");
 };
 template <typename real>
 struct LinBuf {
@@ -150,7 +154,7 @@
 template <typename real>
 struct LinVec {
     real dx[2][32], du[2][32];
-    real zero[64];
+    real zero[128];
 };
 
 template <typename real>
@@ -158,23 +162,40 @@
     using I = LinImg<real>;
     const char *p[2][I::NI];
     unsigned step[I::NI];
+    unsigned skip;
 
     static DEV int piece(int j, int lane)
     {
         const int o = 16 * (64 * j + lane);
         return o < I::END ? o : I::END - 16;
     }
-    DEV void init(const Params &pr, const Bufs &d, const size_t (&b)[2], int s, int kc, int lane)
+    static DEV int rec_of(int q)
     {
+        if constexpr (sizeof(real) == 4) return q;
+        constexpr int A = LQ_CEND * 8, B = A + LQ_BLK_END * 8, C = B + LQ_BLK_END * 8;
+        return q < A ? q : q < B ? q + (LQ_BLK - LQ_CEND) * 8 : q < C ? q + (LQ_BLK + LQ_BLKW - LQ_CEND - LQ_BLK_END) * 8
+                                                                      : q + (LQ_LX - LQ_CEND - 2 * LQ_BLK_END) * 8;
+    }
+    DEV void init(const Params &pr, const Bufs &d, const size_t (&b)[2], int s, int kc, int lane, const int (&cm)[2])
+    {
+        skip = 0;
 #pragma unroll
         for (int j = 0; j < I::NI; ++j) {
             const int o = piece(j, lane);
-            step[j] = o < I::LQ ? KCW * sizeof(real) : o < I::D ? Prec<real>::LQS * sizeof(real) : o < I::DU ? NX * sizeof(real) : NX * 8;
+            const bool lqp = o < I::K;
+            const int ro = rec_of(lqp ? o - I::LQ : 0);
+            if (sizeof(real) == 8 && pr.lq_skip && lqp && ro >= LQ_BLK * 8 && ro < LQ_LX * 8) {
+                const int blk = ro >= (LQ_BLK + LQ_BLKW) * 8;
+#pragma unroll
+                for (int h = 0; h < 2; ++h)
+                    if (lq_block_skipped(cm[h], blk)) skip |= 1u << (h * I::NI + j);
+            }
+            step[j] = o < I::K ? Prec<real>::LQS * sizeof(real) : o < I::D ? KCW * sizeof(real) : o < I::DU ? NX * sizeof(real) : NX * 8;
 #pragma unroll
             for (int h = 0; h < 2; ++h) {
                 const size_t kq = b[h] * pr.Kc + kc;
-                const char *base = o < I::LQ ? (const char *)(Prec<real>::K(d) + kq * KCW) - I::K
-                                 : o < I::D  ? (const char *)(Prec<real>::lq(d) + kq * Prec<real>::LQS) - I::LQ
+                const char *base = o < I::K  ? (const char *)(Prec<real>::lq(d) + kq * Prec<real>::LQS) + (ro - o)
+                                 : o < I::D  ? (const char *)(Prec<real>::K(d) + kq * KCW) - I::K
                                  : o < I::DU ? (const char *)(Prec<real>::def(d, (int)b[h]) + (b[h] * pr.S + s + 1) * NX) - I::D
                                              : (const char *)(d.dU + kq * NX) - I::DU;
                 p[h][j] = base + o;
@@ -194,11 +215,34 @@
 template <typename real>
 DEV void lin_fetch(LinBuf<real> &buf, const LinSrc<real> &src)
 {
+    using I = LinImg<real>;
 #pragma unroll
     for (int h = 0; h < 2; ++h)
 #pragma unroll
-        for (int j = 0; j < LinImg<real>::NI; ++j)
-            lds_dma16_nt(src.p[h][j], (unsigned)(size_t)(buf.v[h] + 1024 * j));
+        for (int j = 0; j < I::NI; ++j) {
+            if (sizeof(real) == 4 || j > 0) {
+                lds_dma16_nt(src.p[h][j], (unsigned)(size_t)(buf.v[h] + 1024 * j));
+            } else if (!((src.skip >> (h * I::NI + j)) & 1u)) {
+                lds_dma16_nt(src.p[h][j], (unsigned)(size_t)(buf.v[h] + 1024 * j));
+            }
+        }
+}
+
+template <typename real>
+DEV void lin_zero_skipped(LinBuf<real> &buf, const LinSrc<real> &src, int lane)
+{
+    using I = LinImg<real>;
+    if constexpr (sizeof(real) == 8) {
+#pragma unroll
+        for (int h = 0; h < 2; ++h)
+#pragma unroll
+            for (int j = 0; j < I::NI; ++j)
+                if ((src.skip >> (h * I::NI + j)) & 1u) {
+                    double2 z;
+                    z.x = 0.0; z.y = 0.0;
+                    *reinterpret_cast<double2 *>(buf.v[h] + 1024 * j + 16 * lane) = z;
+                }
+    }
 }
 
 template <int W>
@@ -251,9 +295,13 @@
     R.use_se = r < 3;
     R.use_sw = r >= 6 && r < 9;
     R.use_rb = r < 12;
-    R.se0 = LQ_SE + 5 * (r < 3 ? r : 0);
+    R.se0 = lq_lin<real>(LQ_SE) + 5 * (r < 3 ? r : 0);
     R.sw0 = r >= 6 && r < 9 ? r - 6 : 0;
-    R.rb0 = LQ_RB + 6 * ((r < 12 ? r : 0) / 3);
+    {
+        constexpr int rb[4] = {lq_lin<real>(rb_at(0, 0)), lq_lin<real>(rb_at(1, 0)), lq_lin<real>(rb_at(2, 0)), lq_lin<real>(rb_at(3, 0))};
+        const int lg = (r < 12 ? r : 0) / 3;
+        R.rb0 = lg == 0 ? rb[0] : lg == 1 ? rb[1] : lg == 2 ? rb[2] : rb[3];
+    }
     const int a = (r < 12 ? r : 0) % 3;
 #pragma unroll
     for (int b = 0; b < 3; ++b) R.rbi[b] = a == 0 ? b : a == 1 ? (b == 0 ? 1 : b == 1 ? 3 : 4) : (b == 0 ? 2 : b == 1 ? 4 : 5);
@@ -327,17 +375,19 @@
     const double *dUi = (const double *)(img + I::DU);
     real *sdxv = S.dx[hf], *sduv = S.du[hf];
     const real *kp = R.cpl ? kimg + R.krow0 : S.zero;
-    const real *sep = R.use_se ? lq + R.se0 : S.zero, *swp = R.use_sw ? lq + LQ_SW + R.sw0 : S.zero;
-    const real *bwp = R.use_sw ? lq + LQ_BW + R.sw0 : S.zero, *rbp = R.use_rb ? lq + R.rb0 : S.zero;
-    const real *lxp = rowl ? lq + LQ_LX : S.zero, *lup = rowl ? lq + LQ_LU : S.zero;
+    const real *sep = R.use_se ? lq + R.se0 : S.zero, *swp = R.use_sw ? lq + R.sw0 : S.zero;
+    const real *bwp = swp, *rbp = R.use_rb ? lq + R.rb0 : S.zero;
+    const real *lxp = rowl ? lq + lq_lin<real>(LQ_LX) : S.zero, *lup = rowl ? lq + lq_lin<real>(LQ_LU) : S.zero;
     real krow[NX], cse[5], csw[17], cbw[12], crb[3];
 #pragma unroll
     for (int c = 0; c < NX; ++c) krow[c] = kp[c];
     const real dUr = (real)dUi[rr];
 #pragma unroll
     for (int q = 0; q < 5; ++q) cse[q] = sep[5 * 0 + q];
-#pragma unroll
-    for (int q = 0; q < 17; ++q) csw[q] = swp[3 * q];
+    static_for<17>([&](auto Q) {
+        constexpr int o = lq_lin<real>(sw_at(0, Q));
+        csw[Q] = swp[o];
+    });
     const real ddr = (rowl ? dd : S.zero)[rr], lxr = lxp[rr], lur = lup[rr];
     if (rowl) sdxv[r] = dx;
     real dxa, dxb;
@@ -355,8 +405,10 @@
     const real du = dUr + (k0 + k1);
     LSTAMP(2);
     SFENCE();
-#pragma unroll
-    for (int q = 0; q < 12; ++q) cbw[q] = bwp[3 * q];
+    static_for<12>([&](auto Q) {
+        constexpr int o = lq_lin<real>(bw_at(0, Q));
+        cbw[Q] = bwp[o];
+    });
 #pragma unroll
     for (int b = 0; b < 3; ++b) crb[b] = rbp[R.rbi[b]];
     if (rowl) sduv[r] = du;
@@ -435,6 +487,7 @@
     const int rr = rowl ? r : 0;
     const real *defg = Prec<real>::def(d, (int)b);
     S.zero[lane] = 0;
+    S.zero[64 + lane] = 0;
     S.dx[hf][r] = 0;
     S.du[hf][r] = 0;
 #if HSDDP_STAMPS
@@ -447,12 +500,15 @@
     LinOut<real> out{};
     for (int i = 0; i < P; ++i) {
         const int N = LY.N(i), s0 = LY.s0(i), k0 = LY.k0(i);
+        LinRow<real> R;
+        int cm[2];
+        load_phase(p, d, eb, hf, i, R.pc, cm);
         LinSrc<real> src;
-        src.init(p, d, eb, s0, k0, lane);
+        src.init(p, d, eb, s0, k0, lane, cm);
         lin_fetch(B0, src);
         out.nprev = 0;
-        LinRow<real> R;
-        load_phase(p, d, eb, hf, i, R.pc);
+        lin_zero_skipped(B0, src, lane);
+        lin_zero_skipped(B1, src, lane);
         if (i > 0) {
             const double *Px = d.term + (b * p.P + (i - 1)) * TW + TM_PX;
             if (rowl) S.dx[hf][r] = dx;
diff --git a/hkd-mpc_amd/csrc/hsddp_lq.hip b/hkd-mpc_amd/csrc/hsddp_lq.hip
--- a/hkd-mpc_amd/csrc/hsddp_lq.hip
+++ b/hkd-mpc_amd/csrc/hsddp_lq.hip
@@ -12,7 +12,7 @@
 template <typename T> constexpr int LQ_STG = 128 / (int)sizeof(T) + 1;
 
 template <typename T>
-DEV void lq_flush(T *wl, const long *ridx, T *lq, int ldw, int lane, int OFF, int N)
+DEV void lq_flush(T *wl, const long *ridx, const int *skip, int sb, T *lq, int ldw, int lane, int OFF, int N)
 {
     wave_sync();
     using T2 = std::conditional_t<std::is_same_v<T, float>, float2, double2>;
@@ -21,7 +21,7 @@
     for (int q = rank; q < 64 * (N / 2); q += na) {
         const int r = q / (N / 2), jp = q % (N / 2);
         const long rr = ridx[r];
-        if (rr >= 0) {
+        if (rr >= 0 && !(skip[r] & sb)) {
             T2 w;
             w.x = wl[r * LQ_STG<T> + 2 * jp];
             w.y = wl[r * LQ_STG<T> + 2 * jp + 1];
@@ -205,37 +205,46 @@
 }
 
 template <typename WT>
-DEV void lq_lu_reb(const Params &p, const WT &w, double mu, const int *c, const double *u, const double *ovr, const double *ur, const double *dl,
-                   const double *ep, double *lu, double *rb)
+DEV void lq_lu(const Params &p, const WT &w, const int *c, const double *u, const double *ur, const double *gu, double *lu)
 {
 #pragma unroll
     for (int j = 0; j < NU; ++j) lu[j] = p.dt * r_diag(w, j) * (u[j] - ur[j]);
-#pragma unroll
-    for (int j = 0; j < 24; ++j) rb[j] = 0.0;
+    if (p.ReB_active) {
+#pragma unroll
+        for (int lg = 0; lg < 4; ++lg)
+            if (c[lg])
+                for (int a = 0; a < 3; ++a) lu[3 * lg + a] += p.dt * gu[3 * lg + a];
+    }
+}
+
+DEV void lq_reb_leg(const Params &p, double mu, const int *c, int lg, const double *u, const double *ovr, const double *dl,
+                    const double *ep, double *gul, double *rb)
+{
+#pragma unroll
+    for (int j = 0; j < 6; ++j) rb[j] = 0.0;
+#pragma unroll
+    for (int j = 0; j < 3; ++j) gul[j] = 0.0;
     auto reb = [&](auto uniform) {
         constexpr bool U = decltype(uniform)::value;
         const double inv_du = p.grf_inv_delta;
-#pragma unroll
-        for (int lg = 0; lg < 4; ++lg) {
-            if (!c[lg]) continue;
-            double gu[3] = {0, 0, 0}, hu[6] = {0, 0, 0, 0, 0, 0};
-            const double f0 = grf_force(u, ovr, 3 * lg), f1 = grf_force(u, ovr, 3 * lg + 1), f2 = grf_force(u, ovr, 3 * lg + 2);
-#pragma unroll
-            for (int r = 0; r < 5; ++r) {
-                double row[3], d1, d2;
-                grf_row(mu, r, row);
-                double g = row[0] * f0 + row[1] * f1 + row[2] * f2;
-                const double dlr = U ? p.grf_delta : dl[5 * lg + r];
-                reb_derivs(g, dlr, U ? inv_du : 1.0 / dlr, d1, d2);
-                double e = U ? p.grf_eps : ep[5 * lg + r];
-                for (int a = 0; a < 3; ++a) gu[a] += e * d1 * row[a];
-                hu[0] += e * (d2 * row[0] * row[0]); hu[1] += e * (d2 * row[0] * row[1]);
-                hu[2] += e * (d2 * row[0] * row[2]); hu[3] += e * (d2 * row[1] * row[1]);
-                hu[4] += e * (d2 * row[1] * row[2]); hu[5] += e * (d2 * row[2] * row[2]);
-            }
-            for (int a = 0; a < 3; ++a) lu[3 * lg + a] += p.dt * gu[a];
-            for (int a = 0; a < 6; ++a) rb[6 * lg + a] = p.dt * hu[a];
-        }
+        if (!c[lg]) return;
+        double gu[3] = {0, 0, 0}, hu[6] = {0, 0, 0, 0, 0, 0};
+        const double f0 = grf_force(u, ovr, 3 * lg), f1 = grf_force(u, ovr, 3 * lg + 1), f2 = grf_force(u, ovr, 3 * lg + 2);
+#pragma unroll
+        for (int r = 0; r < 5; ++r) {
+            double row[3], d1, d2;
+            grf_row(mu, r, row);
+            double g = row[0] * f0 + row[1] * f1 + row[2] * f2;
+            const double dlr = U ? p.grf_delta : dl[5 * lg + r];
+            reb_derivs(g, dlr, U ? inv_du : 1.0 / dlr, d1, d2);
+            double e = U ? p.grf_eps : ep[5 * lg + r];
+            for (int a = 0; a < 3; ++a) gu[a] += e * d1 * row[a];
+            hu[0] += e * (d2 * row[0] * row[0]); hu[1] += e * (d2 * row[0] * row[1]);
+            hu[2] += e * (d2 * row[0] * row[2]); hu[3] += e * (d2 * row[1] * row[1]);
+            hu[4] += e * (d2 * row[1] * row[2]); hu[5] += e * (d2 * row[2] * row[2]);
+        }
+        for (int a = 0; a < 3; ++a) gul[a] = gu[a];
+        for (int a = 0; a < 6; ++a) rb[a] = p.dt * hu[a];
     };
     if (p.ReB_active) {
         if (p.reb_uniform) reb(std::true_type{});
@@ -264,6 +273,7 @@
     __shared__ __attribute__((aligned(16))) char lds[STG > TRM ? STG : TRM];
     T (*stage)[64 * LQ_STG<T>] = reinterpret_cast<T (*)[64 * LQ_STG<T>]>(lds);
     __shared__ long sridx[4][64];
+    __shared__ int sskip[4][64];
     const int lane = threadIdx.x & 63, w = threadIdx.x >> 6;
     constexpr bool BY_KNOT = !SLOTS && !F32;
     const long nunit = (long)p.B * (BY_KNOT ? p.Kc : p.S);
@@ -273,6 +283,7 @@
         return;
     }
     sridx[w][lane] = -1;
+    sskip[w][lane] = 0;
     const long gid = (long)blockIdx.x * blockDim.x + threadIdx.x;
     if (gid >= nunit) return;
     const int b = (int)(gid / (BY_KNOT ? p.Kc : p.S));
@@ -313,6 +324,7 @@
     if (k == L.N(i)) return;
     const int kc = L.k0(i) + k;
     sridx[w][lane] = (long)b * p.Kc + kc;
+    if (!F32 && p.lq_skip) sskip[w][lane] = lq_skip_bits((c[0] != 0) | (c[1] != 0) << 1 | (c[2] != 0) << 2 | (c[3] != 0) << 3);
     double u[NU];
     const double *ug = ubuf(d, wb) + ((size_t)b * p.Kc + kc) * NU;
 #pragma unroll
@@ -332,18 +344,39 @@
     double cd[4] = {(double)c[0], (double)c[1], (double)c[2], (double)c[3]};
     T *wl = stage[w];
     constexpr int W = 128 / (int)sizeof(T);
-    auto col = [&](int pos) -> T & { return wl[lane * LQ_STG<T> + (pos & (W - 1))]; };
     auto put = [&](int pos, double v) {
-        col(pos) = (T)v;
-        if ((pos & (W - 1)) == W - 1) lq_flush(wl, sridx[w], lqT, ldw, lane, pos - (W - 1), W);
+        const int q = lq_rec<T>(pos);
+        if (q < 0) return;
+        wl[lane * LQ_STG<T> + (q & (W - 1))] = (T)v;
+        if ((q & (W - 1)) == W - 1) {
+            const int blk = (q - LQ_BLK) / LQ_BLKW;
+            const int sb = F32 || q < LQ_BLK || q >= LQ_LX ? 0 : 1 << blk;
+            lq_flush(wl, sridx[w], sskip[w], sb, lqT, ldw, lane, q - (W - 1), W);
+        }
     };
-    col(15) = 0;
+    double gu[12];
     hkd_partial_emit(x, u, cd, p.dt, [&](int piece, int j, double v) {
-        const int pos = piece == 0 ? LQ_SE + j : piece == 1 ? sw_at(j / 17, j % 17) : bw_at(j / 12, j % 12);
-        col(pos) = (T)v;
-        if (pos < 96 && ((pos & (W - 1)) == W - 1 || (W == 16 && pos == 14))) {
-            lq_flush(wl, sridx[w], lqT, ldw, lane, pos & ~(W - 1), W);
-            if (pos == 63) col(67) = 0;
+        if (piece == 0) {
+            put(LQ_SE + j, v);
+            if (j == 14) put(LQ_SE + 15, 0.0);
+        } else if (piece == 1) {
+            put(sw_at(j / 17, j % 17), v);
+            if (j == 2 * 17 + 8)
+#pragma unroll
+                for (int q = sw_at(2, 8) + 1; q < LQ_BLK; ++q) put(q, 0.0);
+        } else if (piece == 2) {
+            put(bw_at(j / 12, j % 12), v);
+        } else if constexpr (!F32) {
+#pragma unroll
+            for (int sl = 0; sl < 2; ++sl) {
+                const int lg = lq_block_leg(j, sl);
+                double rb[6];
+                lq_reb_leg(p, mu, c, lg, u, ovr, dl, ep, gu + 3 * lg, rb);
+#pragma unroll
+                for (int e = 0; e < 6; ++e) put(rb_at(lg, e), rb[e]);
+            }
+#pragma unroll
+            for (int q = lq_block_at(j) + LQ_BLK_END; q < lq_block_at(j) + LQ_BLKW; ++q) put(q, 0.0);
         }
     });
     {
@@ -360,15 +393,68 @@
 #pragma unroll
         for (int j = 0; j < NX; ++j) put(LQ_LX + j, lx[j]);
     }
-    double lu[NU], rb[24];
-    lq_lu_reb(p, wr, mu, c, u, ovr, ur, dl, ep, lu, rb);
+#pragma unroll
+    for (int j = 12; j < NU; ++j) u[j] = ug[j];
+    double rbh[F32 ? 24 : 1];
+    if constexpr (F32) {
+#pragma unroll
+        for (int n = 0; n < 4; ++n) {
+            const int lg = n == 0 ? 0 : n == 1 ? 3 : n == 2 ? 1 : 2;
+            double g3[3], r6[6];
+            lq_reb_leg(p, mu, c, lg, u, ovr, dl, ep, g3, r6);
+#pragma unroll
+            for (int a = 0; a < 3; ++a) gu[3 * lg + a] = g3[a];
+#pragma unroll
+            for (int e = 0; e < 6; ++e) rbh[6 * n + e] = r6[e];
+        }
+    }
+    double lu[NU];
+    lq_lu(p, wr, c, u, ur, gu, lu);
 #pragma unroll
     for (int j = 0; j < NU; ++j) put(LQ_LU + j, lu[j]);
-#pragma unroll
-    for (int j = 0; j < 24; ++j) put(LQ_RB + j, rb[j]);
-    if constexpr (F32)
-#pragma unroll
-        for (int j = LQW; j < LQW32; ++j) put(j, 0.0);
+    if constexpr (F32) {
+        auto tail = [&](int q, T v) {
+            wl[lane * LQ_STG<T> + (q & (W - 1))] = v;
+            if ((q & (W - 1)) == W - 1) lq_flush(wl, sridx[w], sskip[w], 0, lqT, ldw, lane, q - (W - 1), W);
+        };
+#pragma unroll
+        for (int j = 0; j < 24; ++j) tail(152 + j, (T)rbh[j]);
+#pragma unroll
+        for (int q = 176; q < LQW32; ++q) tail(q, (T)0);
+        static_assert(!F32 || (lq_pos32(rb_at(0, 0)) == 152 && lq_pos32(rb_at(3, 0)) == 158 && lq_pos32(rb_at(1, 0)) == 164 &&
+                               lq_pos32(rb_at(2, 0)) == 170 && lq_pos32(LQ_LU + 23) == 151), "fp32 record tail");
+    }
+}
+
+template <bool EL>
+__global__ __launch_bounds__(256) void k_lq_zero_blocks(Params p, Bufs d)
+{
+    constexpr int PCS = LQ_BLKW / 2;
+    const long gid = (long)blockIdx.x * blockDim.x + threadIdx.x;
+    const long rec = gid / (2 * PCS);
+    if (rec >= (long)p.B * p.Kc) return;
+    const int q = (int)(gid % (2 * PCS)), blk = q / PCS;
+    const int b = (int)(rec / p.Kc), kc0 = (int)(rec % p.Kc);
+    const auto L = layout_of<EL>(d, b);
+    int i, k;
+    knot_phase(L, kc0, i, k);
+    if (k >= L.N(i)) return;
+    int c[4], cn[4];
+    load_contacts(d, p, b, i, c, cn);
+    const int cmask = (c[0] != 0) | (c[1] != 0) << 1 | (c[2] != 0) << 2 | (c[3] != 0) << 3;
+    if (!lq_block_skipped(cmask, blk)) return;
+    double2 z;
+    z.x = 0.0; z.y = 0.0;
+    *reinterpret_cast<double2 *>(d.lq + ((size_t)b * p.Kc + L.k0(i) + k) * LQW + lq_block_at(blk) + 2 * (q % PCS)) = z;
+}
+
+void launch_lq_zero_blocks(const Params &p, const Bufs &d, hipStream_t st)
+{
+    if (p.fp32 || !p.lq_skip) return;
+    const dim3 g(blocks_for((long)p.B * p.Kc * LQ_BLKW, 256));
+    with_flags([&](auto el) {
+        hipLaunchKernelGGL(k_lq_zero_blocks<decltype(el)::value>, g, dim3(256), 0, st, p, d);
+    }, p.elem_layout);
 }
 
 template <bool EL, typename... TR>
diff --git a/hkd-mpc_amd/csrc/hsddp_lq_layout.h b/hkd-mpc_amd/csrc/hsddp_lq_layout.h
--- /dev/null
+++ b/hkd-mpc_amd/csrc/hsddp_lq_layout.h
@@ -0,0 +1,162 @@
+#pragma once
+
+namespace hsddp {
+
+constexpr int LQ_LINE = 16;
+constexpr int LQ_SE = 0;
+constexpr int LQ_SW = 16;
+constexpr int LQ_CEND = 44;
+constexpr int LQ_BLK = 48;
+constexpr int LQ_BLKW = 48;
+constexpr int LQ_BLK_CF = 30;
+constexpr int LQ_BLK_RB = 30;
+constexpr int LQ_BLK_END = 42;
+constexpr int LQ_LX = 144;
+constexpr int LQ_LU = 168;
+constexpr int LQW = 192;
+constexpr int LQW32 = 192;
+
+constexpr int lq_leg_block(int l) { return (l == 0 || l == 3) ? 0 : 1; }
+constexpr int lq_leg_slot(int l) { return l >= 2 ? 1 : 0; }
+constexpr int lq_block_leg(int blk, int slot) { return blk == 0 ? (slot ? 3 : 0) : (slot ? 2 : 1); }
+constexpr int lq_block_at(int blk) { return LQ_BLK + LQ_BLKW * blk; }
+constexpr int lq_block_legs(int blk) { return blk == 0 ? 0x9 : 0x6; }
+constexpr bool lq_block_skipped(int cmask, int blk) { return (cmask & lq_block_legs(blk)) == 0; }
+constexpr int lq_skip_bits(int cmask) { return (lq_block_skipped(cmask, 0) ? 1 : 0) | (lq_block_skipped(cmask, 1) ? 2 : 0); }
+
+constexpr int sw_at(int r, int q)
+{
+    return q < 9 ? LQ_SW + 3 * q + r
+                 : lq_block_at(lq_leg_block((q - 9) / 2)) + 15 * lq_leg_slot((q - 9) / 2) + 3 * ((q - 9) % 2) + r;
+}
+constexpr int bw_at(int r, int k) { return lq_block_at(lq_leg_block(k / 3)) + 15 * lq_leg_slot(k / 3) + 6 + 3 * (k % 3) + r; }
+constexpr int rb_at(int l, int e) { return lq_block_at(lq_leg_block(l)) + LQ_BLK_RB + 6 * lq_leg_slot(l) + e; }
+
+constexpr int V_SE = LQ_SE, V_D = 104, V_LX = 128, V_LU = 152, V_RB = 176, VW = 200;
+struct LqRange { int rec, len, img; };
+constexpr int V_NR = 6;
+constexpr LqRange V_RANGE[V_NR] = {
+    {0, LQ_CEND, 0},
+    {lq_block_at(0), LQ_BLK_CF, LQ_CEND},
+    {lq_block_at(1), LQ_BLK_CF, LQ_CEND + LQ_BLK_CF},
+    {LQ_LX, 48, V_LX},
+    {lq_block_at(0) + LQ_BLK_RB, 12, V_RB},
+    {lq_block_at(1) + LQ_BLK_RB, 12, V_RB + 12},
+};
+constexpr int lq_img_of(int pos)
+{
+    if (pos < LQ_BLK) return pos < LQ_CEND ? pos : -1;
+    if (pos >= LQ_LX) return pos - LQ_LX + V_LX;
+    const int b = (pos - LQ_BLK) / LQ_BLKW, o = (pos - LQ_BLK) % LQ_BLKW;
+    return o < LQ_BLK_CF ? LQ_CEND + LQ_BLK_CF * b + o : o < LQ_BLK_END ? V_RB + 12 * b + (o - LQ_BLK_RB) : -1;
+}
+constexpr int lq_rec_of_img(int v)
+{
+    for (int i = 0; i < V_NR; ++i)
+        if (v >= V_RANGE[i].img && v < V_RANGE[i].img + V_RANGE[i].len) return v - V_RANGE[i].img + V_RANGE[i].rec;
+    return -1;
+}
+
+constexpr int lq_img_src(int v)
+{
+    return v < LQ_CEND ? v
+         : v < LQ_CEND + LQ_BLK_CF ? v + (LQ_BLK - LQ_CEND)
+         : v < V_D ? v + (LQ_BLK + LQ_BLKW - LQ_CEND - LQ_BLK_CF)
+         : v < V_RB ? v + (LQ_LX - V_LX)
+         : v < V_RB + 12 ? v + (LQ_BLK + LQ_BLK_RB - V_RB)
+                         : v + (LQ_BLK + LQ_BLKW + LQ_BLK_RB - V_RB - 12);
+}
+constexpr int lq_pos32(int pos) { return lq_img_of(pos) < 0 ? -1 : lq_img_of(pos) < V_D ? lq_img_of(pos) : lq_img_of(pos) - 24; }
+template <typename real>
+constexpr int lq_rec(int pos) { return sizeof(real) == 4 ? lq_pos32(pos) : pos; }
+
+constexpr int LIN_LQW = 176;
+constexpr int LIN_NR = 4;
+constexpr LqRange LIN_RANGE[LIN_NR] = {
+    {0, LQ_CEND, 0},
+    {lq_block_at(0), LQ_BLK_END, LQ_CEND},
+    {lq_block_at(1), LQ_BLK_END, LQ_CEND + LQ_BLK_END},
+    {LQ_LX, 48, LQ_CEND + 2 * LQ_BLK_END},
+};
+constexpr int lq_lin_of(int pos)
+{
+    if (pos < LQ_BLK) return pos < LQ_CEND ? pos : -1;
+    if (pos >= LQ_LX) return pos - LQ_LX + LQ_CEND + 2 * LQ_BLK_END;
+    const int b = (pos - LQ_BLK) / LQ_BLKW, o = (pos - LQ_BLK) % LQ_BLKW;
+    return o < LQ_BLK_END ? LQ_CEND + LQ_BLK_END * b + o : -1;
+}
+constexpr int lq_rec_of_lin(int v)
+{
+    for (int i = 0; i < LIN_NR; ++i)
+        if (v >= LIN_RANGE[i].img && v < LIN_RANGE[i].img + LIN_RANGE[i].len) return v - LIN_RANGE[i].img + LIN_RANGE[i].rec;
+    return -1;
+}
+template <typename real>
+constexpr int lq_lin(int pos) { return sizeof(real) == 4 ? lq_pos32(pos) : lq_lin_of(pos); }
+constexpr int lq_lin_block(int v) { return v >= LIN_RANGE[1].img && v < LIN_RANGE[3].img ? (v >= LIN_RANGE[2].img ? 1 : 0) : -1; }
+
+namespace lq_check {
+constexpr bool ranges_16_bytes(const LqRange *r, int n)
+{
+    for (int i = 0; i < n; ++i)
+        if (r[i].rec % 2 || r[i].len % 2 || r[i].img % 2) return false;
+    return true;
+}
+constexpr bool maps_match_ranges()
+{
+    for (int pos = 0; pos < LQW; ++pos) {
+        int v = -1, w = -1;
+        for (int i = 0; i < V_NR; ++i)
+            if (pos >= V_RANGE[i].rec && pos < V_RANGE[i].rec + V_RANGE[i].len) v = pos - V_RANGE[i].rec + V_RANGE[i].img;
+        for (int i = 0; i < LIN_NR; ++i)
+            if (pos >= LIN_RANGE[i].rec && pos < LIN_RANGE[i].rec + LIN_RANGE[i].len) w = pos - LIN_RANGE[i].rec + LIN_RANGE[i].img;
+        if (lq_img_of(pos) != v || lq_lin_of(pos) != w) return false;
+    }
+    return true;
+}
+constexpr bool src_matches_ranges()
+{
+    for (int v = 0; v < VW; ++v)
+        if ((v < V_D || v >= V_LX) && lq_img_src(v) != lq_rec_of_img(v)) return false;
+    return true;
+}
+constexpr bool coefficients_in_reach()
+{
+    for (int r = 0; r < 3; ++r) {
+        for (int q = 0; q < 17; ++q)
+            if (lq_img_of(sw_at(r, q)) < 0 || lq_img_of(sw_at(r, q)) >= V_D) return false;
+        for (int k = 0; k < 12; ++k)
+            if (lq_img_of(bw_at(r, k)) < 0 || lq_img_of(bw_at(r, k)) >= V_D) return false;
+    }
+    return lq_img_of(LQ_SE + 14) < V_D;
+}
+constexpr bool blocks_hold_their_legs()
+{
+    for (int l = 0; l < 4; ++l) {
+        const int lo = lq_block_at(lq_leg_block(l)), hi = lo + LQ_BLK_END;
+        for (int r = 0; r < 3; ++r) {
+            for (int k = 0; k < 2; ++k)
+                if (sw_at(r, 9 + 2 * l + k) < lo || sw_at(r, 9 + 2 * l + k) >= hi) return false;
+            for (int k = 0; k < 3; ++k)
+                if (bw_at(r, 3 * l + k) < lo || bw_at(r, 3 * l + k) >= hi) return false;
+        }
+        for (int e = 0; e < 6; ++e)
+            if (rb_at(l, e) < lo || rb_at(l, e) >= hi) return false;
+    }
+    for (int q = 0; q < 9; ++q)
+        if (sw_at(2, q) >= LQ_CEND) return false;
+    return true;
+}
+}
+static_assert(LQ_BLK % LQ_LINE == 0 && LQ_BLKW % LQ_LINE == 0 && LQ_LX % LQ_LINE == 0 && LQW % LQ_LINE == 0 &&
+              LQ_BLK + 2 * LQ_BLKW == LQ_LX && LQ_LU + 24 == LQW, "record layout: the blocks are whole lines");
+static_assert(LQ_SE + 15 < LQ_SW && sw_at(2, 8) + 1 < LQ_CEND && LQ_CEND <= LQ_BLK && LQ_BLK_END <= LQ_BLKW, "record layout");
+static_assert(lq_check::ranges_16_bytes(V_RANGE, V_NR) && lq_check::ranges_16_bytes(LIN_RANGE, LIN_NR) && V_D % 2 == 0,
+              "every image piece is 16 bytes");
+static_assert(LQ_CEND + 2 * LQ_BLK_CF == V_D && V_D + 24 == V_LX && V_LX + 24 == V_LU && V_LU + 24 == V_RB &&
+              V_RB + 24 == VW && V_D + 24 <= 8 * 16, "image layout: coefficients and Defect in 8 registers' reach");
+static_assert(lq_check::src_matches_ranges() && lq_check::maps_match_ranges(), "the closed-form maps are V_RANGE / LIN_RANGE");
+static_assert(lq_check::coefficients_in_reach() && lq_check::blocks_hold_their_legs(), "record layout");
+static_assert(LQ_CEND + 2 * LQ_BLK_END + 48 == LIN_LQW, "linear image");
+
+}
diff --git a/hkd-mpc_amd/csrc/hsddp_solve.cpp b/hkd-mpc_amd/csrc/hsddp_solve.cpp
--- a/hkd-mpc_amd/csrc/hsddp_solve.cpp
+++ b/hkd-mpc_amd/csrc/hsddp_solve.cpp
@@ -97,6 +97,7 @@
 {
     if (h->p.trace) hipMemsetAsync(h->d.dbg, 0, (size_t)h->p.B * 16 * sizeof(unsigned long long), h->stream);
     sync_ref_columns(h);
+    if (!h->slots_fresh) launch_lq_zero_blocks(h->p, h->d, h->stream);
     launch_reset_elements(h->p, h->d, h->stream);
     launch_rollout(h->p, h->d, 0.0, 0, 1, -1, budget_of(h), terrain_of(h), weights_of(h), h->stream);
     launch_decide(h->p, h->d, 0.0, 0, 1, -1, budget_of(h), terrain_of(h), weights_of(h), h->stream);
@@ -317,6 +318,7 @@
     hipEvent_t e0 = start_stats(h, stats);
     const std::vector<double> trials = ls_steps(h->opt.alpha);
     sync_ref_columns(h);
+    if (!h->slots_fresh) launch_lq_zero_blocks(h->p, h->d, h->stream);
     for (int i = 0; i < n; ++i) iteration_launches(h, trials, tm);
     return finish_stats(h, tm, e0, stats, n, 0, n);
 }
diff --git a/hkd-mpc_amd/csrc/hsddp_sweep.hip b/hkd-mpc_amd/csrc/hsddp_sweep.hip
--- a/hkd-mpc_amd/csrc/hsddp_sweep.hip
+++ b/hkd-mpc_amd/csrc/hsddp_sweep.hip
@@ -52,8 +52,8 @@
 constexpr int MS = 26;
 constexpr int TS = 14;
 constexpr int WS = 25;
-constexpr int V_SE = LQ_SE, V_D = 104, V_LX = 128, V_LU = 152, V_RB = 176, VW = 200;
-static_assert(LQ_BW + 36 == V_D && LQ_LX + 24 == V_LX && LQ_LU + 24 == V_LU && LQ_RB + 24 == V_RB, "image layout");
+constexpr int v_sw(int r, int q) { return lq_img_of(sw_at(r, q)); }
+constexpr int v_bw(int r, int k) { return lq_img_of(bw_at(r, k)); }
 
 template <typename real>
 struct alignas(16) Lds {
@@ -88,9 +88,14 @@
 template <typename real>
 struct Pieces {
     static constexpr int E = 16 / sizeof(real);
-    static constexpr int NA = V_D / E, ND = NX / E, NR = (LQW - V_D) / E, NP = NA + ND + NR;
+    static constexpr int NA = V_D / E, ND = NX / E, NR = (VW - V_D - NX) / E, NP = NA + ND + NR;
     static constexpr int NI = (2 * NP + 63) / 64;
     static_assert(NP * E == VW && V_D % E == 0, "16-byte pieces");
+    static DEV int src(int q)
+    {
+        if constexpr (sizeof(real) == 4) return q < NA ? E * q : E * (q - ND);
+        else return lq_img_src(E * q);
+    }
 };
 
 template <typename real> struct Prec;
@@ -183,8 +188,7 @@
         if (n < 2 * PC::NP) {
             const int e = n >= PC::NP, q = n - e * PC::NP;
             const real *rec = e ? rec1 : rec0, *def = e ? def1 : def0;
-            const real *src = q < PC::NA ? rec + PC::E * q : q < PC::NA + PC::ND ? def + PC::E * (q - PC::NA)
-                                                                                 : rec + PC::E * (q - PC::ND);
+            const real *src = q >= PC::NA && q < PC::NA + PC::ND ? def + PC::E * (q - PC::NA) : rec + PC::src(q);
             lds_dma16(src, (unsigned)(size_t)(&S.img[0][0]) + 1024u * t);
         }
     }
@@ -203,8 +207,7 @@
         if (t < PC::NI && n < 2 * PC::NP) {
             const int e = n >= PC::NP, qq = n - e * PC::NP;
             const real *rec = e ? rec1 : rec0, *def = e ? def1 : def0;
-            const real *src = qq < PC::NA ? rec + PC::E * qq : qq < PC::NA + PC::ND ? def + PC::E * (qq - PC::NA)
-                                                                                    : rec + PC::E * (qq - PC::ND);
+            const real *src = qq >= PC::NA && qq < PC::NA + PC::ND ? def + PC::E * (qq - PC::NA) : rec + PC::src(qq);
             lds_dma16(src, (unsigned)(size_t)(&S.img[q][0][0]) + 1024u * t);
         }
     }
@@ -243,7 +246,7 @@
     auto sw_row = [&](auto I) {
         constexpr int i = I;
         static_for<17>([&](auto Q) {
-            if constexpr (cs_mine<W>(sw_col(Q)) && sw_live<MASK>(Q)) vfma<sw_at(i, Q)>(acc[sw_col(Q)], cf, x[6 + i]);
+            if constexpr (cs_mine<W>(sw_col(Q)) && sw_live<MASK>(Q)) vfma<v_sw(i, Q)>(acc[sw_col(Q)], cf, x[6 + i]);
         });
     };
     auto se_row = [&](auto I) {
@@ -274,13 +277,13 @@
     for (int q = Q0; q < Q1; ++q)
         if (stance<MASK>(q / 3)) acc[q] = __builtin_fma(y9[q % 3], bv[q / 3], acc[q]);
     static_for<Q1 - Q0>([&](auto Q) {
-        if constexpr (stance<MASK>((Q0 + Q) / 3)) vfma<bw_at(0, Q0 + Q)>(acc[Q0 + Q], cf, y6);
+        if constexpr (stance<MASK>((Q0 + Q) / 3)) vfma<v_bw(0, Q0 + Q)>(acc[Q0 + Q], cf, y6);
     });
     static_for<Q1 - Q0>([&](auto Q) {
-        if constexpr (stance<MASK>((Q0 + Q) / 3)) vfma<bw_at(1, Q0 + Q)>(acc[Q0 + Q], cf, y7);
+        if constexpr (stance<MASK>((Q0 + Q) / 3)) vfma<v_bw(1, Q0 + Q)>(acc[Q0 + Q], cf, y7);
     });
     static_for<Q1 - Q0>([&](auto Q) {
-        if constexpr (stance<MASK>((Q0 + Q) / 3)) vfma<bw_at(2, Q0 + Q)>(acc[Q0 + Q], cf, y8);
+        if constexpr (stance<MASK>((Q0 + Q) / 3)) vfma<v_bw(2, Q0 + Q)>(acc[Q0 + Q], cf, y8);
     });
 }
 
@@ -858,7 +861,7 @@
     L.qlane = L.pos < HC;
     const int lq = (L.qlane ? L.pos : 0) / 3, aq = L.pos % 3;
 #pragma unroll
-    for (int a = 0; a < 3; ++a) L.rb[a] = V_RB + 6 * lq + rb_index(aq, a);
+    for (int a = 0; a < 3; ++a) L.rb[a] = V_RB + 6 * (2 * lq_leg_block(lq) + lq_leg_slot(lq)) + rb_index(aq, a);
     L.xkind = (L.pp >= 3 && L.pp < 6) ? 1 : (L.pp >= 12 && L.pp < NX) ? 2 : 0;
     L.xc0 = L.xkind == 1 ? 12 + (L.pp - 3) : L.xkind == 2 ? 3 + (L.pp - 12) % 3 : MS - 1;
     return L;
```
